# junliu111/CV-MonoSLAM

Measured on AMD Instinct MI355X. Metric: srukf_updates_per_sec, higher is better.
Workload: dtype f64; 1 GPU; BASELINE configs[2]: 200 inverse-depth landmarks (n=1204, Na=1209, L=2419), M=N matched, fp64, one batched refactor per frame, synthetic 640x480 figure-8 sequence; landmarks=200, state_dim=1204, sequences_per_gpu=1, update_mode=batched

## Files before the change

cv-monoslam_amd/csrc/srukf_api.hip:

```cpp

#include "srukf_ctx.h"
using namespace srukf_impl;


namespace srukf_impl {

void srukf_pool_init()
{
    static std::mutex mu;
    static unsigned long long done_mask = 0;
    int dev = 0; hipMemPool_t pool = nullptr;
    if (hipGetDevice(&dev) != hipSuccess || dev < 0 || dev >= 64) return;
    const unsigned long long bit = 1ull << dev;
    std::lock_guard<std::mutex> lk(mu);
    if (done_mask & bit) return;
    if (hipDeviceGetDefaultMemPool(&pool, dev) == hipSuccess && pool) {
        unsigned long long keep = ~0ull;
        hipMemPoolSetAttribute(pool, hipMemPoolAttrReleaseThreshold, &keep);
    }
    done_mask |= bit;
}

hipError_t srukf_dmalloc_raw(void** p, size_t bytes)
{
// ... 97 lines not shown
}

void host_weights(int Na, const srukf_params& p, KWeights& w)
{
    const double alpha = p.ut_alpha, beta = p.ut_beta;
    const double Lammda = alpha * alpha * Na - Na;
    switch (p.weight_type) {
    case 0:
        w.wm0 = 1.0 - Na / 3.0; w.wc0 = 1.0 - Na / 3.0; w.wi = (1.0 - w.wc0) / (2 * Na); w.wi_sr = sqrt(w.wi);
        w.gamma = sqrt(Na / (1.0 - w.wm0));
        break;
    case 1:
        w.gamma = sqrt(Na + Lammda); w.wm0 = Lammda / (Na + Lammda); w.wc0 = w.wm0 + (1 - alpha * alpha + beta);
        w.wi = 1.0 / (2 * (Na + Lammda)); w.wi_sr = sqrt(fabs(w.wi));
        break;
    default:
        w.gamma = sqrt(3.0 * Na / 2.0); w.wm0 = 1.0 / 3.0; w.wc0 = 1.0 / 3.0; w.wi = 1.0 / (3.0 * Na); w.wi_sr = sqrt(w.wi);
        break;
    }
}

void prof_collect(srukf_ctx* c)
{
    for (auto& e : c->pev) {
        float ms = 0.f;
        hipEventSynchronize(e.b);
        hipEventElapsedTime(&ms, e.a, e.b);
        c->prof_ms[e.kc] += ms; c->prof_n[e.kc] += 1;
        hipEventDestroy(e.a); hipEventDestroy(e.b);
    }
    c->pev.clear();
}

}


namespace srukf_impl {

std::vector<int> build_tile_table(int n_own, int n_other, bool upper, bool own_is_row, int k_index )
{
    std::vector<std::vector<int>> lst(8);
    for (int x = 0; x < 8; x++)
        for (int o = 0; o < n_other; o++)
            for (int w = x; w < n_own; w += 8) {
                const int r = own_is_row ? w : o, c = own_is_row ? o : w;
                if (upper && c < r) continue;
                lst[x].push_back(r); lst[x].push_back(c);
            }
    {
        for (auto& l : lst) {
            std::vector<std::pair<int, int>> t;
            for (size_t q = 0; q < l.size() / 2; q++) t.push_back({ l[2 * q], l[2 * q + 1] });
            std::stable_sort(t.begin(), t.end(), [k_index](const std::pair<int, int>& a, const std::pair<int, int>& b) {
                return k_index ? a.second > b.second : a.first > b.first; });
            for (size_t q = 0; q < t.size(); q++) { l[2 * q] = t[q].first; l[2 * q + 1] = t[q].second; }
        }
    }
    size_t mx = 0;
    for (auto& l : lst) mx = l.size() / 2 > mx ? l.size() / 2 : mx;
    std::vector<int> tab(mx * 8 * 2, -1);
    for (int x = 0; x < 8; x++)
        for (size_t q = 0; q < lst[x].size() / 2; q++) { tab[(q * 8 + x) * 2] = lst[x][2 * q]; tab[(q * 8 + x) * 2 + 1] = lst[x][2 * q + 1]; }
    return tab;
}

}

static int alloc_zero(srukf_ctx* c, void** p, size_t bytes)
{
    HIPCHK(c, srukf_dmalloc_on(p, bytes, c->stream));
    HIPCHK(c, hipMemsetAsync(*p, 0, bytes, c->stream));
    return SRUKF_OK;
}

#define ALLOC(ptr, count) do { int rc_ = alloc_zero(c, (void**)&(ptr), sizeof(*(ptr)) * (size_t)(count)); if (rc_) { g_create_error = c->err; srukf_destroy(c); return rc_; } } while (0)

static int block_cov(srukf_ctx* c, int off, int bs, double* out)
{
    srukf_launch_block_cov(c->stream, c->d, c->S, off, bs, c->small, nullptr);
    HIPCHK(c, hipMemcpyAsync(c->hstage, c->small, sizeof(double) * bs * bs, hipMemcpyDeviceToHost, c->stream));
    HIPCHK(c, hipStreamSynchronize(c->stream));
    memcpy(out, c->hstage, sizeof(double) * bs * bs);
    return SRUKF_OK;
}

extern "C" {

int srukf_abi_version(void) { return SRUKF_ABI_VERSION; }

int srukf_default_params(srukf_params* p)
{
    if (!p) return SRUKF_ERR_BAD_ARG;
    memset(p, 0, sizeof *p);
    p->cam_dx = 0.0028; p->cam_dy = 0.0028; p->cam_cx = 310.1129; p->cam_cy = 236.7526;
    p->cam_k1 = 0.0001; p->cam_k2 = 0.0; p->cam_f = 2.1735; p->image_w = 640; p->image_h = 480;
    p->a1 = p->a2 = p->a3 = p->a4 = 8.0; p->sigma_measure = 3.0; p->rho0 = 1.0 / 3.0; p->sigma_rho = p->rho0 / 2.0;
    p->sigma_x = 0.02; p->sigma_y = 0.02; p->sigma_z = 0.005; p->sigma_theta = 0.02;
    p->epsilon = 1e-13; p->ut_alpha = 1e-3; p->ut_beta = 2.0;
    p->weight_type = 0; p->noise_type = 0; p->newton_iters = 100;
    return SRUKF_OK;
}

const char* srukf_last_error(const srukf_ctx* ctx) { return ctx ? ctx->err.c_str() : g_create_error.c_str(); }

int srukf_create(srukf_ctx** out, int N, const srukf_params* p, int device, void* stream)
{
    if (!out || !p || N < 0) { g_create_error = "bad argument"; return SRUKF_ERR_BAD_ARG; }
    if (N > 32 * SRUKF_STAT_GROUPS) { g_create_error = "more than 2048 landmarks: the per-group statistics counters (FrameScalars::stat_cnt) serve 64 groups of 32"; return SRUKF_ERR_UNSUPPORTED; }
    if (p->noise_type != 0) { g_create_error = "noise_type != 0 draws random numbers (SLAM.cpp:1505-1516) and is not built"; return SRUKF_ERR_UNSUPPORTED; }
    int ndev = 0;
    if (hipGetDeviceCount(&ndev) != hipSuccess || ndev <= 0 || device < 0 || device >= ndev) {
        g_create_error = "no HIP device (this library has no CPU fallback)";
        return SRUKF_ERR_NO_DEVICE;
    }
    if (hipSetDevice(device) != hipSuccess) { g_create_error = "hipSetDevice failed"; return SRUKF_ERR_NO_DEVICE; }
    hipDeviceProp_t prop;
    if (hipGetDeviceProperties(&prop, device) != hipSuccess) { g_create_error = "hipGetDeviceProperties failed"; return SRUKF_ERR_NO_DEVICE; }
    if (strncmp(prop.gcnArchName, "gfx950", 6) != 0) {
        g_create_error = std::string("device is ") + prop.gcnArchName + ", kernels are built for gfx950 only";
        return SRUKF_ERR_NO_DEVICE;
    }
    srukf_ctx* c = new srukf_ctx();
    c->device = device; c->p = *p;
    if (!g_dbg_graphs) c->use_graph = false;
    memset(c->prof_ms, 0, sizeof c->prof_ms); memset(c->prof_n, 0, sizeof c->prof_n);
    memset(c->prof_flops, 0, sizeof c->prof_flops); memset(c->prof_bytes, 0, sizeof c->prof_bytes);
    if (stream) { c->stream = (hipStream_t)stream; c->own_stream = false; }
    else {
        if (hipStreamCreateWithFlags(&c->stream, hipStreamNonBlocking) != hipSuccess) { g_create_error = "hipStreamCreate failed"; delete c; return SRUKF_ERR_HIP; }
        c->own_stream = true;
    }
    KDims& d = c->d;
    d.N = N; d.n = 6 * N + 4; d.Na = d.n + 5; d.L = 2 * d.Na + 1;
    d.np = round_up(d.n, SRUKF_PAD); d.mp = round_up(2 * N > 0 ? 2 * N : 1, SRUKF_PAD);
    host_weights(d.Na, c->p, c->w);
    const size_t np = d.np, mp = d.mp;
    ALLOC(c->X, np); ALLOC(c->S, np * np); ALLOC(c->G, np * np); ALLOC(c->Gbak, np * np); ALLOC(c->Wf, np * np);
    ALLOC(c->sigR, (size_t)d.L * 8 + 8); ALLOC(c->mpart, srukf_meas_part_doubles(d.mp)); ALLOC(c->dxp, srukf_gain_part_doubles(d.np)); ALLOC(c->Cmat, (np + 64) * 4); ALLOC(c->Z, (size_t)d.L * mp); ALLOC(c->DZ, np * mp);
    ALLOC(c->Ut, mp * np); ALLOC(c->PxyR, 5 * mp);
    { const size_t Nn = (size_t)(N > 0 ? N : 1); ALLOC(c->h, mp + 4 * Nn + (Nn + 1) / 2); c->Si = c->h + mp; c->vis = (int*)(c->h + mp + 4 * Nn);
      ALLOC(c->zcur, mp + (Nn + 1) / 2); c->mcur = (int*)(c->zcur + mp); }
    ALLOC(c->D, np); ALLOC(c->odocur, 8); ALLOC(c->small, 64);
    ALLOC(c->theta, np); ALLOC(c->fs, 1);
    { char* pb0 = nullptr; char* pb1 = nullptr; ALLOC(pb0, srukf_gmw_panel_bytes()); ALLOC(pb1, srukf_gmw_panel_bytes()); c->pan[0] = pb0; c->pan[1] = pb1; }
    { const int rcg = gmw_plan_create(c->gplan, d.np, c->stream); if (rcg) { g_create_error = "persistent GMW resources: allocation failed"; srukf_destroy(c); return rcg; } }
    split_ensure(c, c->gplan);
    {
        std::vector<int> ts = build_tile_table(d.np / 32, d.np / 32, true, true, 0);
        std::vector<int> tp = build_tile_table(d.np / 32, d.mp / 32, false, false, 1);
        c->n_syrk_tiles = (int)ts.size() / 2; c->n_pxy_tiles = (int)tp.size() / 2;
        ALLOC(c->syrk_tiles, ts.size()); ALLOC(c->pxy_tiles, tp.size());
        std::vector<int> th;
        const int hd = srukf_gmw_head_rows(), hx = hd + 64 * srukf_gmw_head_extra_diag();
        for (int pass = 0; pass < 2; pass++)
            for (size_t q = 0; q + 1 < ts.size(); q += 2) {
                if (!(ts[q] >= 0 && (ts[q] * 32 < hd || (ts[q] * 32 < hx && ts[q + 1] * 32 < hx)))) continue;
                const bool crit = ts[q] * 32 < 128 && ts[q + 1] * 32 < 128;
                if (crit == (pass == 0)) { th.push_back(ts[q]); th.push_back(ts[q + 1]); }
            }
        c->n_syrk_head_crit = 0;
        for (size_t q = 0; q + 1 < th.size(); q += 2) if (th[q] * 32 < 128 && th[q + 1] * 32 < 128) c->n_syrk_head_crit++;
        c->n_syrk_head_tiles = (int)th.size() / 2;
        ALLOC(c->syrk_head_tiles, th.size() ? th.size() : 2);
        {
            std::vector<int> qx[8], tb;
            for (size_t q = 0; q + 1 < th.size(); q += 2) { const int x = (th[q + 1] / 2) % 8; qx[x].push_back(th[q]); qx[x].push_back(th[q + 1]); }
            size_t longest = 0;
            for (int x = 0; x < 8; x++) longest = std::max(longest, qx[x].size() / 2);
            for (size_t rnd = 0; rnd < longest; rnd++)
                for (int x = 0; x < 8; x++) { tb.push_back(2 * rnd + 1 < qx[x].size() ? qx[x][2 * rnd] : -1); tb.push_back(2 * rnd + 1 < qx[x].size() ? qx[x][2 * rnd + 1] : -1); }
            c->n_syrk_head_tiles_b = (int)tb.size() / 2;
            ALLOC(c->syrk_head_tiles_b, tb.size() ? tb.size() : 2);
            if (!tb.empty() && hipMemcpyAsync(c->syrk_head_tiles_b, tb.data(), sizeof(int) * tb.size(), hipMemcpyHostToDevice, c->stream) != hipSuccess) {
                g_create_error = "tile table upload failed"; srukf_destroy(c); return SRUKF_ERR_HIP;
            }
            if (hipStreamSynchronize(c->stream) != hipSuccess) { g_create_error = "tile table upload failed"; srukf_destroy(c); return SRUKF_ERR_HIP; }
        }
        if (!th.empty() && hipMemcpyAsync(c->syrk_head_tiles, th.data(), sizeof(int) * th.size(), hipMemcpyHostToDevice, c->stream) != hipSuccess) {
            g_create_error = "tile table upload failed"; srukf_destroy(c); return SRUKF_ERR_HIP;
        }
        if (hipMemcpyAsync(c->syrk_tiles, ts.data(), sizeof(int) * ts.size(), hipMemcpyHostToDevice, c->stream) != hipSuccess ||
            hipMemcpyAsync(c->pxy_tiles, tp.data(), sizeof(int) * tp.size(), hipMemcpyHostToDevice, c->stream) != hipSuccess ||
            hipStreamSynchronize(c->stream) != hipSuccess) {
            g_create_error = "tile table upload failed"; srukf_destroy(c); return SRUKF_ERR_HIP;
        }
    }
    c->hstage_bytes = sizeof(double) * (np * np + 4096);
    if (g_spare_stage && g_spare_stage_bytes >= c->hstage_bytes) {
        c->hstage = g_spare_stage; c->hstage_bytes = g_spare_stage_bytes; g_spare_stage = nullptr; g_spare_stage_bytes = 0;
    }
    if ((!c->hstage && hipHostMalloc((void**)&c->hstage, c->hstage_bytes) != hipSuccess) || hipHostMalloc((void**)&c->hfs, sizeof(FrameScalars) + sizeof(double) * (40 + c->d.mp + 5 * (size_t)c->d.N + 8)) != hipSuccess) {
        g_create_error = "hipHostMalloc failed"; srukf_destroy(c); return SRUKF_ERR_NOMEM;
    }
    memset(c->hfs, 0, sizeof(FrameScalars) + sizeof(double) * 40);
    c->hmeas = (double*)((char*)c->hfs + sizeof(FrameScalars) + sizeof(double) * 40);
    int rc = srukf_reset(c);
    if (rc) { g_create_error = c->err; srukf_destroy(c); return rc; }
    srukf_warm_exact_path(c->stream, c->fs);
    *out = c;
    return SRUKF_OK;
}

int srukf_destroy(srukf_ctx* c)
{
    if (!c) return SRUKF_OK;
    hipSetDevice(c->device);
    for (srukf_ctx* r : c->retired) srukf_destroy(r);
    c->retired.clear();
    if (c->spare_stage) { hipHostFree(c->spare_stage); c->spare_stage = nullptr; c->spare_stage_bytes = 0; }
    batch_plan_forget(c);
    if (c->stream) hipStreamSynchronize(c->stream);
    if (c->ck_stream) hipStreamSynchronize(c->ck_stream);
    if (c->side) hipStreamSynchronize(c->side);
    prof_collect(c);
    if (c->graph_exec) hipGraphExecDestroy(c->graph_exec);
    if (c->graph) hipGraphDestroy(c->graph);
    if (c->graph8_exec) hipGraphExecDestroy(c->graph8_exec);
    if (c->graph8) hipGraphDestroy(c->graph8);
    if (c->graphN_exec) hipGraphExecDestroy(c->graphN_exec);
    if (c->graphN) hipGraphDestroy(c->graphN);
    void* bufs[] = { c->X, c->S, c->G, c->Gbak, c->Wf, c->sigR, c->Cmat, c->Z, c->DZ, c->Ut, c->h , c->PxyR, c->D,
                     c->zcur , c->odocur, c->small, c->theta, c->fs, c->odo_seq, c->z_seq, c->m_seq, c->pan[0], c->pan[1], c->mpart, c->dxp, c->syrk_tiles, c->pxy_tiles, c->syrk_head_tiles,
                     c->perm, c->iperm, c->Sdis, c->ckS, c->ckX, c->ckS2, c->ckX2, c->odo_step, c->export_cnt, c->red_perm, c->red_iperm, c->gdiag, c->red_syrk_tiles, c->syrk_head_tiles_b, c->red_head0_tiles, c->split_fold_list, c->shadowA, c->Utp, c->P1, c->pxy2_tiles, c->nskip, c->slabW, c->slabL, c->gsW, c->gsL, c->S32, c->X32, c->U32, c->mx_part, c->mx_tasks, c->mx_tiles, c->fold_sync, c->dxk, c->A32, c->mxr_part, c->mxr_tasks, c->mxr_tiles, c->mxr_f64_tiles, c->mxr_xt, c->app_patch, c->app_tmpl, c->d_image, c->appR, c->appT, c->appPx, c->corr, c->has_app };
    for (void* b : bufs) if (b) srukf_dfree_on(b, c->stream);
    det_scratch_free(c->det, c->stream);
    gmw_plan_destroy(c->gplan, c->stream);
    gmw_plan_destroy(c->gplan_red, c->stream);
    if (c->side) { hipStreamSynchronize(c->side); hipStreamDestroy(c->side); hipEventDestroy(c->ev_fork); hipEventDestroy(c->ev_join); }
    if (c->ck_stream) { hipStreamSynchronize(c->ck_stream); hipStreamDestroy(c->ck_stream); hipEventDestroy(c->ck_e1); hipEventDestroy(c->ck_e2); if (c->ck_e3) hipEventDestroy(c->ck_e3); }
    if (c->own_stream && c->stream) hipStreamSynchronize(c->stream);
    if (c->hstage) {
        if (!g_spare_stage || g_spare_stage_bytes < c->hstage_bytes) { if (g_spare_stage) hipHostFree(g_spare_stage); g_spare_stage = c->hstage; g_spare_stage_bytes = c->hstage_bytes; }
        else hipHostFree(c->hstage);
    }
    if (c->hfs) hipHostFree(c->hfs);
    if (c->hview) hipHostFree(c->hview);
    if (c->own_stream && c->stream) hipStreamDestroy(c->stream);
    delete c;
    return SRUKF_OK;
}

}

namespace srukf_impl {

void ctx_retire(srukf_ctx* handle, srukf_ctx* old)
{
    drop_graphs(old);
    old->own_stream = false;
    if (old->hstage) {
        if (!handle->spare_stage || handle->spare_stage_bytes < old->hstage_bytes) {
            if (handle->spare_stage) hipHostFree(handle->spare_stage);
            handle->spare_stage = old->hstage; handle->spare_stage_bytes = old->hstage_bytes;
        } else hipHostFree(old->hstage);
        old->hstage = nullptr; old->hstage_bytes = 0;
    }
    handle->retired.push_back(old);
    const double ctx_bytes = 14.0 * 8.0 * (double)old->d.np * old->d.np;
    const size_t keep = (size_t)std::min((double)g_dbg_ctx_keep.load(), std::max(4.0, 16e9 / ctx_bytes));
    while (handle->retired.size() > keep) { srukf_destroy(handle->retired.front()); handle->retired.erase(handle->retired.begin()); }
}

static int ctx_revive(srukf_ctx* r)
{
    if (r->ck_stream) HIPCHK(r, hipStreamSynchronize(r->ck_stream));
    if (r->side) HIPCHK(r, hipStreamSynchronize(r->side));
    r->ck_pending = false; r->ck3_inflight = false; r->ck_valid = false;
    if (r->odo_seq) { srukf_dfree_on(r->odo_seq, r->stream); srukf_dfree_on(r->z_seq, r->stream); srukf_dfree_on(r->m_seq, r->stream); r->odo_seq = nullptr; r->z_seq = nullptr; r->m_seq = nullptr; }
    r->seqF = 0;
    r->storage = SRUKF_STORAGE_F64;
    r->K_new = 0; r->dx_pending = false; r->dx_lm = false; r->xr1_pending = false;
    if (r->fold_sync) HIPCHK(r, hipMemsetAsync(r->fold_sync, 0, sizeof(unsigned int) * (size_t)srukf_fold_words(r->d.mp / 64, r->d.np / 64), r->stream));
    r->null_canonical = false; r->tail_ok = false;
    r->clamp_frame_host = r->clamp_row_host = -1;
    r->next_odo_valid = false; r->fs_seq_step = false; r->last_update_sequential = false;
    r->step_export_attached = false; r->step_export = StepExport{}; r->mirror_next = false; r->meas_seq = 0;
    r->view_auto = false; r->view_unused = 0; r->view_hits = 0;
    r->step_fast_frames = r->step_slow_frames = 0; r->exact_frames = 0;
    r->profiling = false; r->pev.clear();
    r->err.clear();
    HIPCHK(r, hipMemsetAsync(r->fs, 0, sizeof(FrameScalars), r->stream));
    return srukf_reset(r);
}

int ctx_obtain(srukf_ctx* handle, srukf_ctx** out, int N)
{
    for (size_t q = 0; q < handle->retired.size(); q++) {
        srukf_ctx* r = handle->retired[q];
        if (r->d.N != N || r->device != handle->device || r->stream != handle->stream || memcmp(&r->p, &handle->p, sizeof(srukf_params)) != 0) continue;
        handle->retired.erase(handle->retired.begin() + (long)q);
        if (!r->hstage) {
            const size_t need = sizeof(double) * ((size_t)r->d.np * r->d.np + 4096);
            if (handle->spare_stage && handle->spare_stage_bytes >= need) { r->hstage = handle->spare_stage; r->hstage_bytes = handle->spare_stage_bytes; handle->spare_stage = nullptr; handle->spare_stage_bytes = 0; }
            else if (hipHostMalloc((void**)&r->hstage, need) == hipSuccess) r->hstage_bytes = need;
            else { r->hstage = nullptr; srukf_destroy(r); break; }
        }
        if (ctx_revive(r) == SRUKF_OK) { *out = r; return SRUKF_OK; }
        srukf_destroy(r);
        break;
    }
    if (handle->spare_stage && !g_spare_stage) { g_spare_stage = handle->spare_stage; g_spare_stage_bytes = handle->spare_stage_bytes; handle->spare_stage = nullptr; handle->spare_stage_bytes = 0; }
    return srukf_create(out, N, &handle->p, handle->device, handle->stream);
}

}

extern "C" {

int srukf_reset(srukf_ctx* c)
{
    if (!c) return SRUKF_ERR_BAD_ARG;
    HIPCHK(c, hipSetDevice(c->device));
    const KDims& d = c->d;
    const size_t np = d.np;
    step_state_replaced(c);
    HIPCHK(c, hipMemsetAsync(c->X, 0, sizeof(double) * np, c->stream));
    HIPCHK(c, hipMemsetAsync(c->S, 0, sizeof(double) * np * np, c->stream));
    double* hs = c->hstage;
    hs[0] = c->p.sigma_x; hs[1] = c->p.sigma_y; hs[2] = c->p.sigma_z; hs[3] = c->p.sigma_theta;
// ... 300 lines not shown
```

cv-monoslam_amd/csrc/srukf_ctx.h:

```cpp
#pragma once
#include <hip/hip_runtime.h>
#include <math.h>
#include <stdio.h>
#include <stdlib.h>
#include <string.h>
#include <string>
#include <cstddef>
#include <vector>
#include <algorithm>
#include <utility>
#include <atomic>
#include <mutex>
#include <map>
#include "srukf_device.h"
#include "srukf_rank.h"

extern "C" {
void srukf_launch_motion(hipStream_t, KDims, KWeights, srukf_params, double*, double*, double*, double*, FrameScalars*, const double*, const double*, RankArgs);
void srukf_launch_project(hipStream_t, KDims, KWeights, srukf_params, const double*, const double*, const double*, double*, double*, const FrameScalars*);
void srukf_launch_meas_stats(hipStream_t, KDims, KWeights, const double*, const double*, const double*, double*, double*, double*, int*, double*);
int srukf_meas_part_doubles(int);
void srukf_launch_gain(hipStream_t, KDims, KWeights, double*, const double*, const double*, const int*, const double*, const double*,
                       const double*, const int*, const int*, FrameScalars*, double*, double*, const double*, RankArgs, const double*, double*,
                       const double*, int, const double*, double, const double*, int, const double*, double*);
void srukf_launch_project_motion(hipStream_t, KDims, KWeights, srukf_params, double*, double*, double*, double*, double*, double*, FrameScalars*, RankArgs);
int srukf_gain_part_doubles(int);
void srukf_launch_traj(hipStream_t, KDims, const double*, const double*, FrameScalars*, double*, int);
void srukf_launch_block_cov(hipStream_t, KDims, const double*, int, int, double*, const double*);
void srukf_launch_project_points(hipStream_t, srukf_params, int, const double*, const double*, const double*, const double*, double*);
void srukf_launch_pxy(hipStream_t, KDims, const double*, const double*, double*, const void*, int, KWeights, MeasArgs);
void srukf_launch_pxy2(hipStream_t, KDims, const double*, const double*, double*, double*, const void*, int, int, KWeights, MeasArgs, GainFold);
int srukf_pxy2_build_tiles(int mp, int np, int kr, int* out);
int srukf_pxy2_split_groups(void);
void srukf_launch_syrk(hipStream_t, KDims, const double*, const double*, int, int, double*, FrameScalars*, const void*, int, const double*, double*, RankArgs, const double*);
void srukf_launch_gmw_step64(hipStream_t, int, int, int, double, double*, const void*, void*, double*, double*, const FrameScalars*);
int srukf_gmw_panel_bytes(void);
int srukf_gmw_sync_bytes(int T);
int srukf_gmw_build_tiles(int T, int Tp, short* out);
int srukf_gmw_persist_workers(int T, int Tp, int max_workers);
void srukf_launch_gmw_persist(hipStream_t, int, int, double, double*, void*, double*, double*, void*, const void*, int, int, void*, const double*, const double*, int, int, int, int, int);
void srukf_launch_gmw_persist_head(hipStream_t, int, int, double, double*, void*, double*, double*, void*, const void*, int, int, void*, const double*, const double*, int, int, int, int, int, const HeadArgs*);
void srukf_launch_gmw_split(hipStream_t, hipStream_t, int, int, double, double*, void*, double*, double*, void*, const void*, int, void*, int, int, double*, double*, int);
void srukf_launch_gmw_split_fold(hipStream_t, hipStream_t, int, int, double, double*, void*, double*, double*, void*, const void*, int, void*, int, int, double*, double*, const double*, const double*, int);
int srukf_gmw_build_fold_list(int T, int Tp, short* out);
int srukf_gmw_fold_head_tile(int tr, int tc, int head_rows);
int srukf_gmw_fold_head_rows(int Tp);
void srukf_gmw_fold_head_override(int v);
void srukf_launch_gmw_split_alone(hipStream_t, int, int, int, double, double*, void*, double*, double*, void*, const void*, int, void*, int, int, double*, double*);
void srukf_launch_row_energy(hipStream_t, int, int, const double*, double*);
void srukf_launch_rank_diag(hipStream_t, int, int, const double*, const int*, double*);
void srukf_launch_rank_expand(hipStream_t, int, int, int, double, const double*, const double*, const int*, const int*, const double*, void*, const double*, int, double*, double*, double*, double, int, KDims, KWeights, srukf_params, double*, double*, int, const StepExport*, double, unsigned int*, int);
void srukf_launch_project_table(hipStream_t, KDims, KWeights, srukf_params, double*, double*, double*, double*, double*, double*, FrameScalars*, RankArgs, NullSkip);
void srukf_launch_sigr_rows(hipStream_t, KDims, KWeights, const double*, const double*, double*, const FrameScalars*, const int*, int);
void srukf_launch_rank_shadow(hipStream_t, int, int, int, const double*, const int*, double*);
void srukf_launch_rank_canon(hipStream_t, int, int, int, double, const int*, double*);
void srukf_launch_rank_round(hipStream_t, int, int, double*);
void srukf_launch_syrk_own(hipStream_t, int, int, const double*, const double*, int, int, int, double*, void*, const void*, int, int);
int srukf_gmw_register_form(int, int, int, int);
int srukf_pxy2_b_per(int, int);
void srukf_launch_pxy2_b(hipStream_t, KDims, const void*, int, const void*, int, int, KWeights, int);
void srukf_launch_gain_b(hipStream_t, KDims, KWeights, const void*, int, int, double);
void srukf_launch_syrk_b(hipStream_t, KDims, const void*, int, const void*, int, int, int, int);
void srukf_launch_syrk_own_b(hipStream_t, int, int, const void*, int, int, int, int, const void*, int, int);
void srukf_launch_gmw_step64_b(hipStream_t, int, int, int, double, const void*, int, int, int);
void srukf_launch_gmw_pivslab_b(hipStream_t, int, int, int, double, const void*, int, int, int);
void srukf_launch_gmw_trail_b(hipStream_t, int, int, const void*, int, int, int, int);
void srukf_launch_rank_expand_b(hipStream_t, int, int, int, double, const void*, int, double, KDims, KWeights, srukf_params);
int srukf_gmw_head_rows(void);
int srukf_gmw_head_extra_diag(void);
void srukf_launch_gmw_check(hipStream_t, int, int, const double*, const double*, FrameScalars*, const double*, int, double*);
void srukf_launch_gmw_col(hipStream_t, int, int, int, double, const double*, double*, double*, unsigned long long*, FrameScalars*, double*);
void srukf_set_exact_right_looking(int on);
void srukf_warm_exact_path(hipStream_t st, FrameScalars* fs);
int srukf_get_exact_right_looking(void);
void srukf_launch_gmw_stats(hipStream_t, int, int, const double*, FrameScalars*);
void srukf_launch_landmarks_cartesian(hipStream_t, KDims, const double*, const double*, double*, double*);
void srukf_launch_aug_map(hipStream_t, srukf_params, int, int, int, int, double, const double*, const double*, const double*, double*);
void srukf_launch_aug_x(hipStream_t, int, int, int, double, double, const double*, const double*, const int*, double*, double*, int, int);
void srukf_launch_aug_build(hipStream_t, int, int, int, int, double, double, const double*, const double*, const double*, double*, int, int, int);
void srukf_launch_gram(hipStream_t, int, int, const double*, double*);
void srukf_launch_warp_patch(hipStream_t, KDims, srukf_params, const double*, const double*, const double*, const double*, const double*, const double*,
                             const unsigned char*, const int*, unsigned char*);
void srukf_launch_associate(hipStream_t, KDims, srukf_params, const unsigned char*, const double*, const double*, const int*, const int*,
                            const unsigned char*, double*, int*, double*);
int srukf_mixed_build_tasks(int np, int ue, short* out_tasks, int* out_tiles, int* ntiles);
int srukf_mixed_build_tasks_red(int np, int ue, int krows, int rows_lim, short* out_tasks, int* out_tiles, int* ntiles);
int srukf_mixed_krows(int r);
void srukf_launch_split_bf3(hipStream_t, int, int, int, int, const double*, void*, size_t);
void srukf_launch_syrk_bf3(hipStream_t, int, int, int, int, int, const void*, size_t, const void*, int, const void*, int, double*, double*, void*);
size_t srukf_mixed_part_bytes(int ntasks);
void srukf_launch_cvt_f32(hipStream_t, size_t, const double*, float*);
void srukf_launch_cvt_robot_cols(hipStream_t, int, int, const double*, float*);
void srukf_launch_gain_dx(hipStream_t, int, int, const double*, double*, const double*);
void srukf_launch_syrk32(hipStream_t, int, int, int, const float*, const float*, const void*, int, const void*, int, double*, double*, void*, int);
int srukf_app_patch_stride(void);
int srukf_app_tmpl_stride(void);
}

#define SRUKF_GRAPH_FRAMES 8
#define SRUKF_MAX_TENANTS 4
#define SRUKF_NULL_ENERGY 1e-12
#ifndef SRUKF_BATCH_GROUPS_MAX
#define SRUKF_BATCH_GROUPS_MAX 4
#endif

enum KClass { KC_MOTION = 0, KC_PROJECT, KC_STATS, KC_PXY, KC_GAIN, KC_SYRK, KC_GMW_TRAIL, KC_GMW_PERSIST, KC_GMW_CHECK,
              KC_GMW_COL, KC_RANK_EXPAND, KC_PROJECT_MOTION, KC_PROJECT_TABLE, KC_PXY2, KC_MISC,
              KC_DET_RESPONSE, KC_DET_CAND, KC_DET_RANK, KC_DET_SELECT, KC_CAPTURE, KC_COUNT };
struct ProfEvent { hipEvent_t a, b; int kc; };

struct GmwPlan { void* pans = nullptr; void* sync = nullptr; void* tiles = nullptr; int ntiles = 0, nreal = 0, T = 0, Tp = 0, workers = -1, tenants = 1, cus = 0; };

struct DetScratch {
    double *resp = nullptr, *cand_r = nullptr; int *cand_pix = nullptr, *sorted = nullptr, *rank = nullptr, *gxy = nullptr, *blk = nullptr; void* hdr = nullptr;
    void *in = nullptr, *out = nullptr; size_t in_bytes = 0, out_bytes = 0;
};

struct srukf_ctx {
    int device = 0;
    hipStream_t stream = nullptr;
    bool own_stream = false;
    srukf_params p;
    KDims d;
    KWeights w;
    double *X = nullptr, *S = nullptr, *G = nullptr, *Gbak = nullptr, *Wf = nullptr;
    double *sigR = nullptr, *Cmat = nullptr, *Z = nullptr, *DZ = nullptr, *Ut = nullptr;
    double *h = nullptr, *Si = nullptr, *PxyR = nullptr, *D = nullptr;
    double *zcur = nullptr, *odocur = nullptr, *small = nullptr, *mpart = nullptr, *dxp = nullptr;
    int *vis = nullptr, *mcur = nullptr;
    unsigned long long* theta = nullptr;
    bool dx_pending = false;
    bool dx_lm = false;
    unsigned int* fold_sync = nullptr; double* dxk = nullptr; int fold_robot_tiles = 0;
    bool xr1_pending = false;
    int K_new = 0;
    unsigned char *app_patch = nullptr, *app_tmpl = nullptr, *d_image = nullptr;
    double *appR = nullptr, *appT = nullptr, *appPx = nullptr, *corr = nullptr;
    int* has_app = nullptr;
    bool frame_valid = false;
    DetScratch det;
    int storage = SRUKF_STORAGE_F64;
    float *S32 = nullptr, *X32 = nullptr;
    float *U32 = nullptr; double* mx_part = nullptr; void *mx_tasks = nullptr, *mx_tiles = nullptr; int mx_ntasks = 0, mx_ntiles = 0;
    float* A32 = nullptr; double* mxr_part = nullptr; void *mxr_tasks = nullptr, *mxr_tiles = nullptr; int mxr_ntasks = 0, mxr_ntiles = 0, mxr_krows = 0, mxr_for_r = 0;
    int* mxr_f64_tiles = nullptr; int mxr_n_f64_tiles = 0;
    unsigned short* mxr_xt = nullptr; size_t mxr_xt_stride = 0; int mxr_ktot = 0;
    int *perm = nullptr, *iperm = nullptr;
    double* Sdis = nullptr;
    void* pan[2] = { nullptr, nullptr };
    GmwPlan gplan;
    int red_r = 0, red_Tp = 0;
    int rank_aware = 1;
    int *red_perm = nullptr, *red_iperm = nullptr;
    double* gdiag = nullptr;
    double *shadowA = nullptr, *Utp = nullptr;
    double *slabW = nullptr, *slabL = nullptr;
    double *gsW = nullptr, *gsL = nullptr; int gs_panels = 0;
    hipStream_t side = nullptr; hipEvent_t ev_fork = nullptr, ev_join = nullptr;
    bool split_off = false;
    double* P1 = nullptr; int* pxy2_tiles = nullptr; int n_pxy2_tiles = 0, pxy2_split_b0 = 0;
    int* nskip = nullptr; int ns_full = 0, ns_null = 0, ns_rows = 0;
    int* red_head0_tiles = nullptr; int n_red_head0_tiles = 0;
    void* split_fold_list = nullptr; int n_split_fold = 0;
    double red_head0_flop = 0.0;
    int* red_syrk_tiles = nullptr; int n_red_syrk_tiles = 0;
    double red_fac_flop = 0, red_own_flop = 0;
    GmwPlan gplan_red;
    int shared_tenants = 2;
    int gmw_shared = 0;
    int debug_allow_mixed = 0;
    struct DbgSwitches {
        int fused_motion = 2;
        int f32_fuse = 1;
        int table_perm = 1;
        int tail_fuse = 1;
        int head_fold = 1;
        int nullskip = 1;
        int pxy2 = 1;
        int step_fuse_export = 1;
        int view_auto = 1;
        int step_early = 2;
        int step_spin = 1;
        int step_fast = 1;
        int split_record = 0;
        int null_canon = 1;
        int split_fold = 1;
        int gain_fold = 0;
        int mixed_rank = 1;
        int mixed_null_ppm = 1;
        int mixed_bf16 = 0;
        int mixed_f64_robot = 1;
    } dbg;
    bool null_canonical = false;
    bool tail_ok = false;
    int debug_starve = 0;
    int clamp_frame_host = -1, clamp_row_host = -1;
    double *ckS = nullptr, *ckX = nullptr;
    int *syrk_tiles = nullptr, *pxy_tiles = nullptr;
    int *syrk_head_tiles = nullptr;
    int n_syrk_tiles = 0, n_pxy_tiles = 0, n_syrk_head_tiles = 0, n_syrk_head_crit = 0;
    int* syrk_head_tiles_b = nullptr; int n_syrk_head_tiles_b = 0;
    FrameScalars* fs = nullptr;
    int seqF = 0;
    double *odo_seq = nullptr, *z_seq = nullptr;
    int* m_seq = nullptr;
    double* hstage = nullptr; size_t hstage_bytes = 0;
    FrameScalars* hfs = nullptr;
    double* hmeas = nullptr;
    int phase = 0;
    double next_odo[6] = { 0, 0, 0, 0, 0, 0 }; bool next_odo_valid = false;
    double* odo_step = nullptr;
    double step_odo[6] = { 0, 0, 0, 0, 0, 0 };
    int step_seqF = 1;
    bool step_fast = false;
    bool step_uncommitted = false;
    bool step_chain = false;
    bool proj_valid = false; double proj_odo[6] = { 0, 0, 0, 0, 0, 0 };
    bool fs_seq_step = false;
    bool last_update_sequential = false;
    double *ckS2 = nullptr, *ckX2 = nullptr; hipEvent_t ck_e3 = nullptr; bool ck_valid = false;
    bool ck3_inflight = false;
    unsigned spin_ok = 0;
    bool pre_issued = false; double pre_odo[6] = { 0, 0, 0, 0, 0, 0 };
    bool next_pose_pending = false;
    bool setstep_done = false; double setstep_odo[6] = { 0, 0, 0, 0, 0, 0 };
    hipStream_t ck_stream = nullptr; hipEvent_t ck_e1 = nullptr, ck_e2 = nullptr; bool ck_pending = false;
    unsigned long long meas_seq = 0;
    bool step_export_attached = false;
    int* export_cnt = nullptr;
    StepExport step_export = {};
    bool mirror_next = false;
    unsigned long long step_seq = 0;
    double* hview = nullptr; size_t hview_doubles = 0;
    bool view_auto = false; int view_unused = 0;
    int view_hits = 0;
    bool view_cached = false;
    bool robot_cached = false;
    bool f32_stale = false;
    int step_fast_frames = 0, step_slow_frames = 0;
    double* spare_stage = nullptr; size_t spare_stage_bytes = 0;
    int split_fold_seqs = 0;
    int fold_seqs = 0;
    int exact_frames = 0;
    bool async_pending = false;
    std::vector<srukf_ctx*> retired;
    std::string err;
    hipGraph_t graph = nullptr, graph8 = nullptr;
    hipGraphExec_t graph_exec = nullptr, graph8_exec = nullptr;
    hipGraph_t graphN = nullptr; hipGraphExec_t graphN_exec = nullptr; int graphN_frames = 0;
    bool use_graph = true;
    bool profiling = false;
    std::vector<ProfEvent> pev;
    double prof_ms[KC_COUNT]; long long prof_n[KC_COUNT]; double prof_flops[KC_COUNT]; double prof_bytes[KC_COUNT];
};

#define HIPCHK(ctx, call) do { hipError_t e_ = (call); if (e_ != hipSuccess) { \
    char b_[256]; snprintf(b_, sizeof b_, "%s failed: %s (%s:%d)", #call, hipGetErrorString(e_), __FILE__, __LINE__); \
    (ctx)->err = b_; return SRUKF_ERR_HIP; } } while (0)

namespace srukf_impl {

inline bool storage_f32_like(const srukf_ctx* c) { return c->storage == SRUKF_STORAGE_F32 || (c->storage == SRUKF_STORAGE_F32_MIXED && c->dbg.mixed_rank && c->A32); }

extern const char* const kclass_name[KC_COUNT];
extern thread_local std::string g_create_error;
extern std::atomic<int> g_dbg_gmw_persist, g_dbg_gmw_fused, g_dbg_rank_fused, g_dbg_rank_fold, g_dbg_rank_aware, g_dbg_graphs, g_dbg_mem_split, g_dbg_shared_tenants;
extern std::atomic<int> g_dbg_batch_wide, g_dbg_batch_groups, g_dbg_batch_split, g_dbg_head_fold_free;
extern std::atomic<int> g_dbg_timing, g_dbg_fold_head, g_dbg_fold_force, g_dbg_ctx_keep, g_dbg_batch_xcd, g_dbg_batch_k128;

inline int round_up(int v, int m) { return (v + m - 1) / m * m; }

void srukf_pool_init();
hipError_t srukf_dmalloc_raw(void** p, size_t bytes);
template <class T> inline hipError_t srukf_dmalloc(T** p, size_t bytes) { return srukf_dmalloc_raw((void**)p, bytes); }
hipError_t srukf_dfree(void* p);
template <class T> inline hipError_t srukf_dmalloc_on(T** p, size_t bytes, hipStream_t st) { srukf_pool_init(); return hipMallocAsync((void**)p, bytes ? bytes : 8, st); }
hipError_t srukf_dfree_on(void* p, hipStream_t st);

void launch_refactor_reset(hipStream_t st, int np, unsigned long long* theta_bits, FrameScalars* fs, int reset_stats);
void launch_set_seq(hipStream_t st, FrameScalars* fs, const double* odo_seq, int seqF, double a1, double a2, double a3, double a4);
void launch_set_frame(hipStream_t st, FrameScalars* fs, int frame, int clear_clamp);
void launch_set_traj(hipStream_t st, FrameScalars* fs, double* traj_base);
void launch_set_run(hipStream_t st, FrameScalars* fs, int frame, int clear_clamp, double* traj_base);
void launch_set_step(hipStream_t st, FrameScalars* fs, double* odo, int seqF, double a1, double a2, double a3, double a4, int fresh, const double poses[9]);
void launch_export(hipStream_t st, const void* a, size_t bytes_a, const void* b, size_t bytes_b, void* host_pinned, unsigned long long* flag = nullptr, unsigned long long seq = 0);
void launch_set_frame_control(hipStream_t st, FrameScalars* fs);
void launch_commit_motion(hipStream_t st, int n, int ld, double* X, double* S, const double* Cm, const FrameScalars* fs, double* A, const int* iperm, int rk);
void launch_sym_permute(hipStream_t st, int n, int ld, const double* src, int lds, double* dst, const int* map);
void launch_gather(hipStream_t st, int n, int ld, const double* src, double* dst, const int* map);
void launch_zero_rows(hipStream_t st, int ld, int r0, double* A);
void launch_quantize(hipStream_t st, int n, int ld, double* S, double* X, float* S32, float* X32);

void gmw_plan_destroy(GmwPlan& g, hipStream_t st = nullptr);
int gmw_plan_create(GmwPlan& g, int np, hipStream_t st, int Tp = 0, int tenants = 1);
void host_weights(int Na, const srukf_params& p, KWeights& w);
std::vector<int> build_tile_table(int n_own, int n_other, bool upper, bool own_is_row, int k_index );
void prof_collect(srukf_ctx* c);
void adopt_context(srukf_ctx* c, srukf_ctx* c2);
int ctx_obtain(srukf_ctx* handle, srukf_ctx** out, int N);
void ctx_retire(srukf_ctx* handle, srukf_ctx* old);

void det_scratch_free(DetScratch& s, hipStream_t st);
int ensure_image(srukf_ctx* c);
int take_frame(srukf_ctx* c, const unsigned char* gray);
void launch_capture_patch(hipStream_t st, const unsigned char* img, int W, int first, int K, const double* uv, const double* X, int n,
                          unsigned char* app_patch, unsigned char* app_tmpl, double* appR, double* appT, double* appPx, int* has_app);

#define SRUKF_LM_RECORD_DOUBLES 113
void launch_lm_record(hipStream_t st, const double* P66, const double* X, int k, double eps, const unsigned char* app_patch, const double* appR,
                      const double* appT, const double* appPx, const int* has_app, double* out);
void launch_lm_insert(hipStream_t st, const double* S, int ld, const double* X, int p6, int L, const double* blk, double* S2, double* X2, int n2, int ld2);

struct ProfScope {
    srukf_ctx* c; int kc; hipEvent_t a = nullptr, b = nullptr;
    ProfScope(srukf_ctx* c_, int kc_, double flops, double bytes) : c(c_), kc(kc_) {
        if (c->profiling) {
            hipEventCreate(&a); hipEventCreate(&b); hipEventRecord(a, c->stream);
            c->prof_flops[kc] += flops; c->prof_bytes[kc] += bytes;
        }
    }
    ~ProfScope() {
        if (c->profiling) { hipEventRecord(b, c->stream); c->pev.push_back({ a, b, kc }); }
    }
};

void step_commit_motion(srukf_ctx* c);
unsigned long long* step_flag(srukf_ctx* c);
int step_wait_export(srukf_ctx* c, unsigned long long seq);
void step_invalidate(srukf_ctx* c);
void step_state_replaced(srukf_ctx* c);
void step_ck_join(srukf_ctx* c);

void quantize_state(srukf_ctx* c);
RankArgs rank_args(const srukf_ctx* c, bool prep_next = false, bool dzperm = false, bool f32round = false);
NullSkip null_skip(const srukf_ctx* c);
const double* take_xr1(srukf_ctx* c);
void seq_predict_fused(srukf_ctx* c, int mode);
void seq_predict_motion(srukf_ctx* c, const double* odo_pair_dev);
void seq_predict_measurement(srukf_ctx* c, bool fused_stats);
void shadow_rebuild(srukf_ctx* c);
bool gmw_plan_persists(const srukf_ctx* c, const GmwPlan& gp);
bool gmw_use_persist(const srukf_ctx* c);
int gmw_persist_mode();
int plan_tenants(const srukf_ctx* c);
int gate_limit(const srukf_ctx* c);
void rank_expand(srukf_ctx* c, bool frame_tail, bool table = false, bool fuse = false);
bool replay_red_fused(const srukf_ctx* c);
bool replay_red_perm(const srukf_ctx* c);
int replay_motion_mode(const srukf_ctx* c);
bool replay_fuse_mode(const srukf_ctx* c);
bool head_fold_ok(const srukf_ctx* c);
int gmw_fused_mode();
int rank_fused_mode();
// ... 29 lines not shown
```

cv-monoslam_amd/csrc/srukf_debug.hip:

```cpp

#include "srukf_ctx.h"
using namespace srukf_impl;


namespace srukf_impl {
std::atomic<int> g_dbg_gmw_persist{1}, g_dbg_gmw_fused{1}, g_dbg_rank_fused{1}, g_dbg_rank_fold{1}, g_dbg_rank_aware{1}, g_dbg_graphs{1};
std::atomic<int> g_dbg_mem_split{1};
std::atomic<int> g_dbg_shared_tenants{2};
std::atomic<int> g_dbg_batch_wide{1}, g_dbg_batch_groups{0}, g_dbg_batch_split{1};
std::atomic<int> g_dbg_timing{0}, g_dbg_fold_head{0}, g_dbg_fold_force{0}, g_dbg_ctx_keep{24}, g_dbg_batch_xcd{1}, g_dbg_batch_k128{1};
std::atomic<int> g_dbg_head_fold_free{0};
}

static bool debug_buffer(srukf_ctx* c, const char* key, double** ptr, long long* cap)
{
    const KDims& d = c->d;
    const GmwPlan& gp = c->red_r > 0 ? c->gplan_red : c->gplan;
    double* src = nullptr; long long n = 0;
    if (!strcmp(key, "Z")) { src = c->Z; n = (long long)d.L * d.mp; }
    else if (!strcmp(key, "DZ")) { src = c->DZ; n = (long long)d.np * d.mp; }
    else if (!strcmp(key, "sigR")) { src = c->sigR; n = (long long)(d.L + 1) * 8; }
    else if (!strcmp(key, "Cmat")) { src = c->Cmat; n = (long long)d.n * 4; }
    else if (!strcmp(key, "Xr1")) { src = (double*)((char*)c->fs + offsetof(FrameScalars, Xr1)); n = 4; }
    else if (!strcmp(key, "Utp")) { src = c->Utp; n = c->Utp ? (long long)d.mp * d.np : 0; }
    else if (!strcmp(key, "P1")) { src = c->P1; n = c->P1 ? (long long)d.mp * d.np : 0; }
    else if (!strcmp(key, "h")) { src = c->h; n = 2LL * d.N; }
    else if (!strcmp(key, "Si")) { src = c->Si; n = 4LL * d.N; }
    else if (!strcmp(key, "det_resp")) { src = c->det.resp; n = c->det.resp ? (long long)c->p.image_w * (long long)c->p.image_h : 0; }
    else if (!strcmp(key, "Wf")) { src = c->Wf; n = (long long)d.np * d.np; }
    else if (!strcmp(key, "Gbak")) { src = c->Gbak; n = (long long)d.np * d.np; }
    else if (!strcmp(key, "G")) { src = c->G; n = (long long)d.np * d.np; }
    else if (!strcmp(key, "D")) { src = c->D; n = d.np; }
    else if (!strcmp(key, "fold_dbg")) { src = c->fold_sync ? (double*)(c->fold_sync + ((srukf_fold_words(d.mp / 64, d.np / 64) + 1) & ~1)) : nullptr; n = c->fold_sync ? FOLD_DBG_STAMPS : 0; }
    else if (!strcmp(key, "gsW")) { src = c->gsW; n = c->gsW ? (long long)c->gs_panels * 64 * d.np : 0; }
    else if (!strcmp(key, "gsL")) { src = c->gsL; n = c->gsL ? (long long)c->gs_panels * 64 * d.np : 0; }
    else if (!strcmp(key, "pans")) { src = (double*)gp.pans; n = gp.pans ? (long long)srukf_gmw_panel_bytes() * gp.T / 8 : 0; }
    else if (!strcmp(key, "sync")) { src = (double*)gp.sync; n = gp.sync ? (long long)srukf_gmw_sync_bytes(gp.T) / 8 : 0; }
    else return false;
    *ptr = src; *cap = n;
    return true;
}

extern "C" {

int srukf_debug_allow_mixed(srukf_ctx* c, int on)
{
    if (!c) return SRUKF_ERR_BAD_ARG;
    c->debug_allow_mixed = on ? 1 : 0;
    return SRUKF_OK;
}

int srukf_debug_poke_state(srukf_ctx* c, int row, int col, double value)
{
    if (!c || row < 0 || col < row || col >= c->d.n) return SRUKF_ERR_BAD_ARG;
    HIPCHK(c, hipSetDevice(c->device));
    step_commit_motion(c); step_invalidate(c);
    HIPCHK(c, hipStreamSynchronize(c->stream));
    HIPCHK(c, hipMemcpy(c->S + (size_t)row * c->d.np + col, &value, sizeof(double), hipMemcpyHostToDevice));
    return SRUKF_OK;
}

int srukf_debug_set(srukf_ctx* c, const char* key, int value)
{
    if (!key) return SRUKF_ERR_BAD_ARG;
    struct { const char* k; std::atomic<int>* v; } globals[] = { { "gmw_persist", &g_dbg_gmw_persist }, { "gmw_fused", &g_dbg_gmw_fused }, { "rank_fused", &g_dbg_rank_fused },
                                                    { "rank_fold", &g_dbg_rank_fold }, { "rank_aware", &g_dbg_rank_aware }, { "graphs", &g_dbg_graphs }, { "mem_split", &g_dbg_mem_split }
                                                  };
    if (!strcmp(key, "batch_split")) { g_dbg_batch_split = value ? 1 : 0; batch_drop_all_graphs(); return SRUKF_OK; }
    if (!strcmp(key, "head_fold_free")) { if (value < 1) return SRUKF_ERR_BAD_ARG; g_dbg_head_fold_free = value; if (c) { hipSetDevice(c->device); step_commit_motion(c); step_invalidate(c); hipStreamSynchronize(c->stream); drop_graphs(c); } return SRUKF_OK; }
    if (!strcmp(key, "batch_groups")) { if (value < 0 || value > SRUKF_BATCH_GROUPS_MAX) return SRUKF_ERR_BAD_ARG; g_dbg_batch_groups = value; return SRUKF_OK; }
    if (!strcmp(key, "batch_wide")) { g_dbg_batch_wide = value ? 1 : 0; return SRUKF_OK; }
    if (!strcmp(key, "timing")) { g_dbg_timing = value ? 1 : 0; return SRUKF_OK; }
    if (!strcmp(key, "fold_head")) { g_dbg_fold_head = value < 0 ? 0 : value; srukf_gmw_fold_head_override(g_dbg_fold_head); return SRUKF_OK; }
    if (!strcmp(key, "batch_k128")) { g_dbg_batch_k128 = value ? 1 : 0; batch_drop_all_graphs(); return SRUKF_OK; }
    if (!strcmp(key, "batch_xcd")) { g_dbg_batch_xcd = value ? 1 : 0; batch_drop_all_graphs(); return SRUKF_OK; }
    if (!strcmp(key, "ctx_keep")) { g_dbg_ctx_keep = value < 0 ? 0 : value; return SRUKF_OK; }
    if (!strcmp(key, "fold_force")) { g_dbg_fold_force = value ? 1 : 0; return SRUKF_OK; }
    if (!strcmp(key, "exact_rl")) { srukf_set_exact_right_looking(value); return SRUKF_OK; }
    if (!strcmp(key, "shared_tenants")) {
        if (value < 2 || value > 8) return SRUKF_ERR_BAD_ARG;
        g_dbg_shared_tenants = value;
        return SRUKF_OK;
    }
    for (auto& g : globals)
        if (!strcmp(key, g.k)) {
            g.v->store(!strcmp(key, "mem_split") ? value : (value ? 1 : 0));
            if (c) { hipSetDevice(c->device); step_commit_motion(c); step_invalidate(c); hipStreamSynchronize(c->stream); drop_graphs(c); if (!strcmp(key, "rank_aware")) return update_null_set(c); }
            return SRUKF_OK;
        }
    if (!c) return SRUKF_ERR_BAD_ARG;
    HIPCHK(c, hipSetDevice(c->device));
    step_commit_motion(c); step_invalidate(c);
    HIPCHK(c, hipStreamSynchronize(c->stream));
    if (!strcmp(key, "use_graph")) c->use_graph = value != 0;
    else if (!strcmp(key, "pxy2")) c->dbg.pxy2 = value ? 1 : 0;
    else if (!strcmp(key, "nullskip")) c->dbg.nullskip = value ? 1 : 0;
    else if (!strcmp(key, "head_fold")) c->dbg.head_fold = value ? 1 : 0;
    else if (!strcmp(key, "tail_fuse")) c->dbg.tail_fuse = value ? 1 : 0;
    else if (!strcmp(key, "table_perm")) c->dbg.table_perm = value ? 1 : 0;
    else if (!strcmp(key, "f32_fuse")) c->dbg.f32_fuse = value ? 1 : 0;
    else if (!strcmp(key, "split_record")) c->dbg.split_record = value ? 1 : 0;
    else if (!strcmp(key, "gain_fold")) c->dbg.gain_fold = value ? 1 : 0;
    else if (!strcmp(key, "null_canon")) c->dbg.null_canon = value ? 1 : 0;
    else if (!strcmp(key, "split_fold")) c->dbg.split_fold = value < 0 ? 0 : value > 2 ? 2 : value;
    else if (!strcmp(key, "mixed_rank")) c->dbg.mixed_rank = value ? 1 : 0;
    else if (!strcmp(key, "mixed_f64_robot")) c->dbg.mixed_f64_robot = value ? 1 : 0;
    else if (!strcmp(key, "mixed_bf16")) c->dbg.mixed_bf16 = value ? 1 : 0;
    else if (!strcmp(key, "mixed_null_ppm")) c->dbg.mixed_null_ppm = value < 0 ? 0 : value;
    else if (!strcmp(key, "step_fast")) c->dbg.step_fast = value ? 1 : 0;
    else if (!strcmp(key, "step_spin")) c->dbg.step_spin = value ? 1 : 0;
    else if (!strcmp(key, "step_early")) c->dbg.step_early = value < 0 ? 0 : value > 2 ? 2 : value;
    else if (!strcmp(key, "view_auto")) { c->dbg.view_auto = value ? 1 : 0; if (!value) { c->view_auto = false; c->view_cached = false; } }
    else if (!strcmp(key, "step_fuse_export")) c->dbg.step_fuse_export = value ? 1 : 0;
    else if (!strcmp(key, "fused_motion")) c->dbg.fused_motion = value < 0 ? 0 : value > 2 ? 2 : value;
    else { c->err = std::string("srukf_debug_set: unknown key ") + key; return SRUKF_ERR_BAD_ARG; }
    drop_graphs(c);
    return SRUKF_OK;
}

int srukf_debug_gmw_stamps(srukf_ctx* c, unsigned long long* buf)
{
    if (!c) return SRUKF_ERR_BAD_ARG;
    static unsigned long long* dbuf = nullptr;
    HIPCHK(c, hipSetDevice(c->device));
    HIPCHK(c, hipStreamSynchronize(c->stream));
    GmwPlan& g = c->red_r > 0 ? c->gplan_red : c->gplan;
    if (!g.sync) return SRUKF_ERR_SEQUENCE;
    if (!dbuf) { HIPCHK(c, hipMalloc((void**)&dbuf, 8 * 4096)); HIPCHK(c, hipMemset(dbuf, 0, 8 * 4096)); }
    if (buf) HIPCHK(c, hipMemcpy(buf, dbuf, 8 * 4096, hipMemcpyDeviceToHost));
    HIPCHK(c, hipMemcpy((char*)g.sync + offsetof(GmwSync, dbg), &dbuf, 8, hipMemcpyHostToDevice));
    return SRUKF_OK;
}

int srukf_debug_get(srukf_ctx* c, const char* key, long long* value)
{
    if (!c || !key || !value) return SRUKF_ERR_BAD_ARG;
    HIPCHK(c, hipSetDevice(c->device));
    HIPCHK(c, hipMemcpyAsync(c->hfs, c->fs, sizeof(FrameScalars), hipMemcpyDeviceToHost, c->stream));
    HIPCHK(c, hipStreamSynchronize(c->stream));
    if (!strcmp(key, "gmw_aborts")) *value = c->hfs->gmw_aborts;
    else if (!strcmp(key, "clamp_rows")) *value = c->hfs->clamp_rows;
    else if (!strcmp(key, "frame")) *value = c->hfs->frame;
    else if (!strcmp(key, "frozen")) *value = c->hfs->frozen;
    else if (!strcmp(key, "gate_timeouts")) *value = c->hfs->gate_timeouts;
    else if (!strcmp(key, "gmw_shared")) *value = c->gmw_shared;
    else if (!strcmp(key, "split_off")) *value = c->split_off ? 1 : 0;
    else if (!strncmp(key, "pad", 3) && key[3] >= '1' && key[3] <= '7' && !key[4]) {
        const GmwPlan& gp = c->red_r > 0 ? c->gplan_red : c->gplan;
        unsigned long long v = 0, zero = 0;
        const size_t off = offsetof(GmwSync, pad) + 8 * (size_t)(key[3] - '0');
        if (gp.sync) { HIPCHK(c, hipMemcpy(&v, (char*)gp.sync + off, sizeof v, hipMemcpyDeviceToHost)); HIPCHK(c, hipMemcpy((char*)gp.sync + off, &zero, sizeof zero, hipMemcpyHostToDevice)); }
        *value = (long long)v;
    }
    else if (!strcmp(key, "abort_code")) {
        const GmwPlan& gp = c->red_r > 0 ? c->gplan_red : c->gplan;
        unsigned long long code = 0, zero = 0;
        if (gp.sync) {
            HIPCHK(c, hipMemcpy(&code, (char*)gp.sync + offsetof(GmwSync, pad), sizeof code, hipMemcpyDeviceToHost));
            HIPCHK(c, hipMemcpy((char*)gp.sync + offsetof(GmwSync, pad), &zero, sizeof zero, hipMemcpyHostToDevice));
        }
        *value = (long long)code;
    }
    else if (!strcmp(key, "step_fast")) *value = c->step_fast_frames;
    else if (!strcmp(key, "step_slow")) *value = c->step_slow_frames;
    else if (!strcmp(key, "exact_frames")) *value = c->exact_frames;
    else if (!strcmp(key, "fold_seqs")) *value = c->fold_seqs;
    else if (!strcmp(key, "split_fold_seqs")) *value = c->split_fold_seqs;
    else if (!strncmp(key, "pxy2_stamp", 10) && key[10] >= '1' && key[10] <= '7') { const unsigned long long* t = (const unsigned long long*)(c->hmeas + c->d.mp + 5 * (size_t)c->d.N); *value = (long long)(t[key[10] - '0'] - t[0]); }
    else if (!strcmp(key, "meas_flag_ticks")) { const unsigned long long* t = (const unsigned long long*)(c->hmeas + c->d.mp + 5 * (size_t)c->d.N); *value = (long long)(t[1] - t[0]); }
    else if (!strcmp(key, "view_hits")) *value = c->view_hits;
    else if (!strcmp(key, "view_auto")) *value = c->view_auto ? 1 : 0;
    else if (!strcmp(key, "split_form")) *value = split_form(c, c->red_r > 0 ? c->gplan_red : c->gplan) ? 1 : 0;
    else if (!strncmp(key, "plan_", 5)) {
        const GmwPlan& gp = c->red_r > 0 ? c->gplan_red : c->gplan;
        const bool persist = gmw_use_persist(c) && gmw_plan_persists(c, gp);
        const char* k = key + 5;
        if (!strcmp(k, "T")) *value = gp.T;
        else if (!strcmp(k, "Tp")) *value = gp.Tp;
        else if (!strcmp(k, "tiles")) *value = gp.nreal;
        else if (!strcmp(k, "workers")) *value = gp.workers;
        else if (!strcmp(k, "persist")) *value = persist ? 1 : 0;
        else if (!strcmp(k, "register_form")) *value = (persist && !split_form(c, gp) && srukf_gmw_register_form(gp.T, gp.Tp, gp.ntiles, gp.workers)) ? 1 : 0;
        else if (!strcmp(k, "tiles_per_worker")) *value = gp.workers > 0 ? (gp.nreal + gp.workers - 1) / gp.workers : -1;
        else if (!strcmp(k, "fold")) *value = replay_red_fused(c) ? 1 : 0;
        else if (!strcmp(k, "head_fold")) *value = (replay_red_fused(c) && head_fold_ok(c)) ? 1 : 0;
        else if (!strcmp(k, "red_perm")) *value = (!replay_red_fused(c) && replay_red_perm(c)) ? 1 : 0;
        else if (!strcmp(k, "motion")) *value = replay_motion_mode(c);
        else if (!strcmp(k, "fuse")) *value = replay_fuse_mode(c) ? 1 : 0;
        else if (!strcmp(k, "kept")) *value = c->red_r;
        else if (!strcmp(k, "sync_doubles")) *value = gp.sync ? srukf_gmw_sync_bytes(gp.T) / 8 : 0;
        else if (!strcmp(k, "pans_doubles")) *value = gp.pans ? (long long)srukf_gmw_panel_bytes() * gp.T / 8 : 0;
        else if (!strcmp(k, "slab_panels")) *value = c->gs_panels;
        else return SRUKF_ERR_BAD_ARG;
    }
    else return SRUKF_ERR_BAD_ARG;
    return SRUKF_OK;
}

int srukf_debug_copy(srukf_ctx* c, const char* key, double* out, long long count)
{
    if (!c || !key || !out || count < 0) return SRUKF_ERR_BAD_ARG;
    HIPCHK(c, hipSetDevice(c->device));
    HIPCHK(c, hipStreamSynchronize(c->stream));
    double* src = nullptr; long long cap = 0;
    if (!debug_buffer(c, key, &src, &cap)) return SRUKF_ERR_BAD_ARG;
    if (!src || count > cap) return SRUKF_ERR_DIM_MISMATCH;
    HIPCHK(c, hipMemcpy(out, src, sizeof(double) * (size_t)count, hipMemcpyDeviceToHost));
    return SRUKF_OK;
}

int srukf_debug_upload(srukf_ctx* c, const char* key, const double* in, long long count)
{
    if (!c || !key || !in || count < 0) return SRUKF_ERR_BAD_ARG;
    HIPCHK(c, hipSetDevice(c->device));
    HIPCHK(c, hipStreamSynchronize(c->stream));
    double* dst = nullptr; long long cap = 0;
    if (!debug_buffer(c, key, &dst, &cap)) return SRUKF_ERR_BAD_ARG;
    if (!dst || count > cap) return SRUKF_ERR_DIM_MISMATCH;
    HIPCHK(c, hipMemcpy(dst, in, sizeof(double) * (size_t)count, hipMemcpyHostToDevice));
    return SRUKF_OK;
}

int srukf_debug_starve_workers(srukf_ctx* c, int on)
{
    if (!c) return SRUKF_ERR_BAD_ARG;
    c->debug_starve = on == 2 ? 2 : on ? 1 : 0;
    step_invalidate(c);
    drop_graphs(c);
    return SRUKF_OK;
}

int srukf_gmw_host(int device, int n, const double* G, double* S_out, double* D_out, double epsilon, int force_slow, int* clamp_hit)
{
    if (n < 1 || !G || !S_out) return SRUKF_ERR_BAD_ARG;
    int ndev = 0;
    if (hipGetDeviceCount(&ndev) != hipSuccess || device < 0 || device >= ndev) return SRUKF_ERR_NO_DEVICE;
    if (hipSetDevice(device) != hipSuccess) return SRUKF_ERR_NO_DEVICE;
    const int np = round_up(n, SRUKF_PAD);
    const size_t bytes = sizeof(double) * (size_t)np * np;
    std::vector<double> hG((size_t)np * np, 0.0), hS((size_t)np * np, 0.0), hD(np, 0.0);
    for (int r = 0; r < n; r++) for (int c = r; c < n; c++) hG[(size_t)r * np + c] = G[(size_t)r * n + c];
    struct Res {
        double *dG = nullptr, *dS = nullptr, *dD = nullptr, *dWf = nullptr; unsigned long long* dTh = nullptr; FrameScalars* dFs = nullptr;
        void* pan[2] = { nullptr, nullptr }; GmwPlan gp;
        ~Res() { for (void* b : { (void*)dG, (void*)dS, (void*)dD, (void*)dWf, (void*)dTh, (void*)dFs, pan[0], pan[1] }) if (b) srukf_dfree(b); gmw_plan_destroy(gp); }
    } r;
#define GH(call) do { if ((call) != hipSuccess) return SRUKF_ERR_HIP; } while (0)
    GH(srukf_dmalloc((void**)&r.dG, bytes)); GH(srukf_dmalloc((void**)&r.dS, bytes)); GH(srukf_dmalloc((void**)&r.dWf, bytes));
    GH(srukf_dmalloc((void**)&r.dD, sizeof(double) * np)); GH(srukf_dmalloc((void**)&r.dTh, sizeof(unsigned long long) * np)); GH(srukf_dmalloc((void**)&r.dFs, sizeof(FrameScalars)));
    GH(hipMemcpy(r.dG, hG.data(), bytes, hipMemcpyHostToDevice));
    GH(hipMemset(r.dS, 0, bytes)); GH(hipMemset(r.dWf, 0, bytes)); GH(hipMemset(r.dTh, 0, sizeof(unsigned long long) * np));
    GH(hipMemset(r.dFs, 0, sizeof(FrameScalars))); GH(hipMemset(r.dD, 0, sizeof(double) * np));
    hipStream_t st = nullptr;
    srukf_launch_gmw_stats(st, n, np, r.dG, r.dFs);
    FrameScalars fs;
    if (!force_slow) {
        if (gmw_persist_mode()) { const int rc = gmw_plan_create(r.gp, np, st); if (rc) return rc; }
        if (gmw_persist_mode() && r.gp.workers >= 0) {
            srukf_launch_gmw_persist(st, n, np, epsilon, r.dG, r.gp.pans, r.dD, r.dS, r.gp.sync, r.gp.tiles, r.gp.ntiles, r.gp.workers, r.dFs, nullptr, nullptr, 0, 0, 0, 0, 0);
        } else {
            GH(srukf_dmalloc(&r.pan[0], srukf_gmw_panel_bytes())); GH(srukf_dmalloc(&r.pan[1], srukf_gmw_panel_bytes()));
            GH(hipMemset(r.pan[0], 0, srukf_gmw_panel_bytes())); GH(hipMemset(r.pan[1], 0, srukf_gmw_panel_bytes()));
            int pb = 0;
            for (int j0 = -64; j0 + 64 < np; j0 += 64, pb ^= 1)
                srukf_launch_gmw_step64(st, n, np, j0, epsilon, r.dG, r.pan[pb ^ 1], r.pan[pb], r.dD, r.dS, nullptr);
        }
        GH(hipDeviceSynchronize());
        srukf_launch_gmw_check(st, n, np, r.dD, r.dS, r.dFs, nullptr, 0, nullptr);
        GH(hipMemcpy(&fs, r.dFs, sizeof fs, hipMemcpyDeviceToHost));
        if (clamp_hit) *clamp_hit = fs.clamp_rows;
        if (fs.clamp_rows > 0) force_slow = 2;
    }
    if (force_slow) {
        GH(hipMemcpy(r.dG, hG.data(), bytes, hipMemcpyHostToDevice));
        GH(hipMemset(r.dTh, 0, sizeof(unsigned long long) * np));
        GH(hipMemset(r.dS, 0, bytes));
        for (int j = 0; j < n; j++) srukf_launch_gmw_col(st, n, np, j, epsilon, r.dG, r.dWf, r.dD, r.dTh, r.dFs, r.dS);
        GH(hipMemcpy(&fs, r.dFs, sizeof fs, hipMemcpyDeviceToHost));
        if (clamp_hit && force_slow == 1) *clamp_hit = fs.clamp_rows;
    }
    GH(hipDeviceSynchronize());
    GH(hipMemcpy(hS.data(), r.dS, bytes, hipMemcpyDeviceToHost));
    GH(hipMemcpy(hD.data(), r.dD, sizeof(double) * np, hipMemcpyDeviceToHost));
#undef GH
    for (int rr = 0; rr < n; rr++) memcpy(S_out + (size_t)rr * n, hS.data() + (size_t)rr * np, sizeof(double) * n);
    if (D_out) memcpy(D_out, hD.data(), sizeof(double) * n);
    return SRUKF_OK;
}

int srukf_project_host(int device, const srukf_params* p, int count, const double* feat6, const double* pos3, const double* psi,
                       const double* err2, double* uv_out)
{
    if (!p || count < 1 || !feat6 || !pos3 || !psi || !err2 || !uv_out) return SRUKF_ERR_BAD_ARG;
    int ndev = 0;
    if (hipGetDeviceCount(&ndev) != hipSuccess || device < 0 || device >= ndev) return SRUKF_ERR_NO_DEVICE;
    if (hipSetDevice(device) != hipSuccess) return SRUKF_ERR_NO_DEVICE;
    double *df, *dp, *ds, *de, *dout;
    srukf_dmalloc((void**)&df, sizeof(double) * 6 * count); srukf_dmalloc((void**)&dp, sizeof(double) * 3 * count);
    srukf_dmalloc((void**)&ds, sizeof(double) * count); srukf_dmalloc((void**)&de, sizeof(double) * 2 * count); srukf_dmalloc((void**)&dout, sizeof(double) * 2 * count);
    hipMemcpy(df, feat6, sizeof(double) * 6 * count, hipMemcpyHostToDevice); hipMemcpy(dp, pos3, sizeof(double) * 3 * count, hipMemcpyHostToDevice);
    hipMemcpy(ds, psi, sizeof(double) * count, hipMemcpyHostToDevice); hipMemcpy(de, err2, sizeof(double) * 2 * count, hipMemcpyHostToDevice);
    srukf_launch_project_points(nullptr, *p, count, df, dp, ds, de, dout);
    hipError_t e = hipDeviceSynchronize();
    hipMemcpy(uv_out, dout, sizeof(double) * 2 * count, hipMemcpyDeviceToHost);
    srukf_dfree(df); srukf_dfree(dp); srukf_dfree(ds); srukf_dfree(de); srukf_dfree(dout);
    return e == hipSuccess ? SRUKF_OK : SRUKF_ERR_HIP;
}

}
```

cv-monoslam_amd/csrc/srukf_device.h:

```cpp
#pragma once
#include <hip/hip_runtime.h>
#include "../../include/srukf.h"

typedef double d4 __attribute__((ext_vector_type(4)));

#define SRUKF_NB 32
#define SRUKF_PAD 64

struct KDims {
    int N, n, Na, L;
    int np, mp;
};

struct KWeights { double wm0, wc0, wi, wi_sr, gamma; };

#define SRUKF_STAT_GROUPS 64
struct FrameScalars {
    double Ut[3];
    double Mt[3];
    double Xr0[4];
    unsigned long long gmax_bits;
    unsigned long long ximax_bits;
    int clamp_rows;
    int clamp_first;
// ... 148 lines not shown
    oy = vis ? vy : 0.0;
}

__device__ __forceinline__ void srukf_sigma_feat(const double (&base)[6], const double (&dev)[6], double e0, double e1, double gq,
                                                 double (&feat)[6], double& q0, double& q1)
{
#pragma clang fp contract(off)
#pragma unroll
    for (int e = 0; e < 6; e++) feat[e] = fma(dev[e], gq, base[e] * 1) + 0;
    q0 = fma(e0, gq, 0.0 * 1) + 0; q1 = fma(e1, gq, 0.0 * 1) + 0;
}
__device__ __forceinline__ void srukf_project_sigma(const srukf_params& p, double f1, double f2, const double (&base)[6], const double (&dev)[6],
                                                    double e0, double e1, double gq, const double* r, double& ox, double& oy)
{
    double feat[6], q0, q1;
    srukf_sigma_feat(base, dev, e0, e1, gq, feat, q0, q1);
    srukf_project(p, f1, f2, feat, r[0], r[1], r[2], r[4], r[5], q0, q1, ox, oy);
}

#define GAIN_SLICES 32
__device__ __forceinline__ void srukf_gain_dx_job(int n, int np, const double* __restrict__ dxp, double* __restrict__ X, int job, const double* xr1 = nullptr, int f32 = 0, int lmN = 0)
{
    const int r = job * 256 + threadIdx.x;
    if (r >= n) return;
    double acc = 0.0;
    if (lmN > 0) {
        const int per = (lmN + GAIN_SLICES - 1) / GAIN_SLICES;
        for (int u = 0; u < GAIN_SLICES; u++) {
            const int kb = u * per, cnt = min(lmN, kb + per) - kb;
            double s[4] = { 0.0, 0.0, 0.0, 0.0 };
            for (int q = 0; q < cnt; q++) s[q & 3] += dxp[(size_t)(kb + q) * np + r];
            acc += (s[0] + s[1]) + (s[2] + s[3]);
        }
    } else
#pragma unroll
    for (int u = 0; u < GAIN_SLICES; u++) acc += dxp[(size_t)u * np + r];
    const double x = (xr1 && r >= n - 4) ? xr1[r - (n - 4)] : X[r];
    double v = x + acc;
    if (f32) v = (double)(float)v;
    X[r] = v;
}

struct GainLm { double i00, i01, i10, i11, y0, y1; int on; };
__device__ __forceinline__ GainLm srukf_gain_lm(double s00, double s01, double s10, double s11, double z0, double z1, double h0, double h1, int on)
{
#pragma clang fp contract(off)
    GainLm g;
    double det = fma(s00, s11, -(s01 * s10));
    g.i00 = 0.0; g.i01 = 0.0; g.i10 = 0.0; g.i11 = 0.0;
    if (det != 0.0) { det = 1.0 / det; g.i00 = s11 * det; g.i01 = -s01 * det; g.i10 = -s10 * det; g.i11 = s00 * det; }
    const double v0 = z0 - h0, v1 = z1 - h1;
    g.y0 = fma(g.i10, v1, g.i00 * v0); g.y1 = fma(g.i11, v1, g.i01 * v0);
    g.on = on;
    return g;
}
__device__ __forceinline__ double srukf_gain_pxy(double q0, double q1, bool split, double dz, bool nullrow, double sqeps, double sc)
{
#pragma clang fp contract(off)
    double q = q0;
    if (split) q = q + q1;
    if (nullrow) q = fma(sqeps, dz, q);
    return sc * q;
}
__device__ __forceinline__ double srukf_gain_recentre(double p, double dxs, double s4, double hz, double rse)
{
#pragma clang fp contract(off)
    return fma(-hz, rse, fma(-dxs, s4, p));
}
__device__ __forceinline__ void srukf_gain_apply(const GainLm& g, double p0, double p1, double& u0, double& u1, double& c)
{
#pragma clang fp contract(off)
    u0 = fma(p1, g.i10, p0 * g.i00);
    u1 = fma(p1, g.i11, p0 * g.i01);
    c = fma(u1, g.y1, u0 * g.y0);
}

struct GainFold {
    unsigned int* sync;
    double* Utp; double* dxk;
    const double* z_seq; const int* m_seq;
    const double* DZp; const int* perm; const int* iperm; int r; int split_b0; double sqeps; double sc;
    double* S; double* A;
    int nmt, nbt, bt_r0, bt_r1, robot_tiles;
};
#define FOLD_FLAG_STRIDE 1024
#define FOLD_PAIR(mt, bt, nbt) (4 * ((mt) * (nbt) + (bt)))
__host__ __device__ inline int srukf_fold_flag_base(int nmt, int nbt) { return (4 * nmt * nbt + FOLD_FLAG_STRIDE - 1) / FOLD_FLAG_STRIDE * FOLD_FLAG_STRIDE; }
#define FOLD_MOTION(nmt, nbt) (srukf_fold_flag_base(nmt, nbt))
#define FOLD_ROBOT(nmt, nbt) (srukf_fold_flag_base(nmt, nbt) + FOLD_FLAG_STRIDE)
#define FOLD_STAT(g, nmt, nbt) (srukf_fold_flag_base(nmt, nbt) + FOLD_FLAG_STRIDE * (2 + (g)))
__host__ __device__ inline int srukf_fold_words(int nmt, int nbt) { return srukf_fold_flag_base(nmt, nbt) + FOLD_FLAG_STRIDE * (2 + SRUKF_STAT_GROUPS); }
#define FOLD_DBG_STAMPS 8192
#ifdef SRUKF_FOLD_DBG
#define FOLD_TS(gf, slot) do { if ((gf).sync && (threadIdx.x & 63) == 0) { unsigned long long t_; asm volatile("s_memrealtime %0\n\ts_waitcnt lgkmcnt(0)" : "=s"(t_) :: "memory"); \
    ((unsigned long long*)((gf).sync + ((srukf_fold_words((gf).nmt, (gf).nbt) + 1) & ~1)))[slot] = t_; } } while (0)
#else
#define FOLD_TS(gf, slot) do { } while (0)
#endif

struct NullSkip { const int* dirs; const int* nulls; const int* rows; int nfull, nnull, nrows; const int* iperm; int r; };

struct MeasArgs {
    const double* X; const double* xrob; const double* sigR; const double* Z; double* part;
    double* h; double* Si; int* vis; double* PxyR;
    FrameScalars* fs; int gx;
    NullSkip ns;
    int preamble;
    int fmode;
    double* Cm;
    char* hmirror; unsigned long long* hflag; unsigned long long hseq;
    unsigned long long* hstamp;
};

struct StepExport { unsigned long long* dst; int nfs; double* view; unsigned long long* flag; unsigned long long seq; int* cnt; int set; double* odo; double poses[6]; double a[4]; };
__device__ __forceinline__ void srukf_step_scalars(FrameScalars* fs, double* odo, int seqF, const double (&a)[4], bool clear_frozen = true)
{
    fs->odo_seq = odo; fs->seqF = seqF;
    fs->a[0] = a[0]; fs->a[1] = a[1]; fs->a[2] = a[2]; fs->a[3] = a[3];
    fs->frame = 0;
    fs->traj_base = nullptr;
    fs->stat_count = 0;
    for (int q = 0; q < SRUKF_STAT_GROUPS; q++) fs->stat_cnt[q] = 0;
    fs->clamp_rows = 0; fs->clamp_first = 0x7fffffff; fs->clamp_frame = 0x7fffffff; fs->gmw_aborts = 0;
    if (clear_frozen) fs->frozen = 0;
}

__device__ __forceinline__ double ld_dev(const double* p) { return __hip_atomic_load(p, __ATOMIC_RELAXED, __HIP_MEMORY_SCOPE_AGENT); }
__device__ __forceinline__ void st_dev(double* p, double v) { __hip_atomic_store(p, v, __ATOMIC_RELAXED, __HIP_MEMORY_SCOPE_AGENT); }
template <bool DEV> __device__ __forceinline__ double ld_g(const double* p) { if constexpr (DEV) return ld_dev(p); else return *p; }
template <bool DEV> __device__ __forceinline__ void st_d4(double* p, d4 v)
{
    if constexpr (DEV) { st_dev(p, v[0]); st_dev(p + 1, v[1]); st_dev(p + 2, v[2]); st_dev(p + 3, v[3]); }
    else *(d4*)p = v;
}

#define GMW_EPOCH_SHIFT 12
#define GMW_FLAG_COPIES 16
#define GMW_FLAG_STRIDE 512
struct GmwSync {
    unsigned long long epoch;
    unsigned int exited;
    int abort;
    unsigned long long* dbg;
    unsigned int head_done;
    unsigned int head_crit;
    unsigned int resident;
    unsigned int pad32;
    unsigned long long pad[59];
    unsigned long long panel_ready[GMW_FLAG_COPIES * GMW_FLAG_STRIDE];
    unsigned long long half_ready[GMW_FLAG_COPIES * GMW_FLAG_STRIDE];
};
__device__ __forceinline__ unsigned int* gmw_head_crit(GmwSync* sy) { return (unsigned int*)&sy->panel_ready[GMW_FLAG_STRIDE / 2]; }
__device__ __forceinline__ unsigned int* gmw_head_done(GmwSync* sy) { return (unsigned int*)&sy->half_ready[GMW_FLAG_STRIDE / 2]; }
__device__ __forceinline__ unsigned long long* gmw_sync_ver(GmwSync* sy) { return (unsigned long long*)(sy + 1); }
#define GMW_VER_STRIDE 16
#define GMW_VIDX(I, J, T) (((size_t)(I) * (T) + (J)) * GMW_VER_STRIDE)
__device__ __forceinline__ unsigned long long* gmw_sync_slabver(GmwSync* sy, int T) { return (unsigned long long*)(sy + 1) + (size_t)T * T * GMW_VER_STRIDE; }
__device__ __forceinline__ unsigned long long* gmw_sync_formver(GmwSync* sy, int T) { return (unsigned long long*)(sy + 1) + (size_t)2 * T * T * GMW_VER_STRIDE; }

#ifdef SRUKF_GMW_DBG
#define GMW_DBG(sy, slot, val) do { if (__builtin_amdgcn_readfirstlane(threadIdx.x >> 6) == 0 && (sy)->dbg) __hip_atomic_store(&(sy)->dbg[blockIdx.x * 8 + (slot)], (unsigned long long)(val), __ATOMIC_RELAXED, __HIP_MEMORY_SCOPE_SYSTEM); } while (0)
#define GMW_DBG2(sy, slot, val) do { if ((sy)->dbg) __hip_atomic_store(&(sy)->dbg[blockIdx.x * 8 + (slot)], (unsigned long long)(val), __ATOMIC_RELAXED, __HIP_MEMORY_SCOPE_SYSTEM); } while (0)
#define GMW_TS(sy, p, slot) do { if ((sy)->dbg) { unsigned long long t_; asm volatile("s_memrealtime %0\n\ts_waitcnt lgkmcnt(0)" : "=s"(t_) :: "memory"); (sy)->dbg[2048 + (p) * 8 + (slot)] = t_; } } while (0)
#else
#define GMW_DBG(sy, slot, val)
#define GMW_DBG2(sy, slot, val)
#define GMW_TS(sy, p, slot)
#endif

#ifdef SRUKF_STAMPS
__device__ unsigned long long srukf_stamps[32];
#define STAMP(i) do { if (blockIdx.x == 0 && blockIdx.y == 0 && threadIdx.x == 0) { unsigned long long t_; asm volatile("s_memtime %0\n\ts_waitcnt lgkmcnt(0)" : "=s"(t_) :: "memory"); srukf_stamps[i] = t_; } } while (0)
#define STAMPW(i) do { if (blockIdx.x == 0 && blockIdx.y == 0 && (threadIdx.x & 63) == 0) { unsigned long long t_; asm volatile("s_memtime %0\n\ts_waitcnt lgkmcnt(0)" : "=s"(t_) :: "memory"); srukf_stamps[i] = t_; } } while (0)
#else
#define STAMP(i)
#define STAMPW(i)
#endif

struct Step64Args { double* G; double* Sout; double* D; void* pan[2]; double* Wb; double* Lb; };
struct SyrkOwnArgs { const double* S0; const double* Ut0; double* G; FrameScalars* fs; };

struct LaunchCtx;
```

cv-monoslam_amd/csrc/srukf_gmw_persist.hip:

```cpp
#include <hip/hip_runtime.h>
#include <algorithm>
#include <cmath>
#include <cstdio>
#include <cstdlib>
#include <utility>
#include <vector>
#include "srukf_device.h"
#include "srukf_tiles.h"
#include "srukf_gmw_cols.h"
#include "srukf_gmw_panel.h"
#include "srukf_rank.h"

#ifndef GMW_XWG_LIMIT
#define GMW_XWG_LIMIT (1 << 16)
#endif
__device__ __forceinline__ unsigned long long gmw_uniform64(unsigned long long v)
{
    return ((unsigned long long)(unsigned)__builtin_amdgcn_readfirstlane((int)(v >> 32)) << 32) | (unsigned)__builtin_amdgcn_readfirstlane((int)v);
}
__device__ __forceinline__ bool gmw_wait_ge(const unsigned long long* f, unsigned long long want, const int* abort_flag)
{
    for (int spins = 0; spins < GMW_XWG_LIMIT; spins++) {
        if (gmw_uniform64(__hip_atomic_load(f, __ATOMIC_RELAXED, __HIP_MEMORY_SCOPE_AGENT)) >= want) return true;
        if ((spins & 31) == 31 && __builtin_amdgcn_readfirstlane(__hip_atomic_load(abort_flag, __ATOMIC_RELAXED, __HIP_MEMORY_SCOPE_AGENT))) return false;
        __builtin_amdgcn_s_sleep(1);
    }
    return false;
}
__device__ __forceinline__ void gmw_abandon(GmwSync* sy, unsigned int site)
{
    __hip_atomic_store(&sy->abort, 1, __ATOMIC_RELAXED, __HIP_MEMORY_SCOPE_AGENT);
    if ((threadIdx.x & 63) == 0) atomicCAS(&sy->pad[0], 0ull, ((unsigned long long)site << 32) | (unsigned long long)(blockIdx.x + 1));
}
__device__ __forceinline__ void gmw_set_flag(unsigned long long* f, unsigned long long v)
{
    __hip_atomic_store(f, v, __ATOMIC_RELAXED, __HIP_MEMORY_SCOPE_AGENT);
}
__device__ __forceinline__ void gmw_set_panel_flag(unsigned long long* f, unsigned long long v, int lane)
{
    if (lane < GMW_FLAG_COPIES) __hip_atomic_store(&f[lane * GMW_FLAG_STRIDE], v, __ATOMIC_RELAXED, __HIP_MEMORY_SCOPE_AGENT);
}
__device__ __forceinline__ void gmw_publish(unsigned long long* f, unsigned long long v, bool wv0)
{
    asm volatile("s_waitcnt vmcnt(0)" ::: "memory");
    __syncthreads();
    if (wv0) gmw_set_flag(f, v);
}

struct GmwPivotKeep {
    double* T1;
    double* T2;
    double* Ep;
    double* rD;
    double* sq;
};

__device__ __forceinline__ void gmw_stage_tile(double (*dst)[G64_LS], const double* __restrict__ G, int ld, int row0, int col0, int lane)
{
    const double* src = G + (size_t)row0 * ld + col0 + lane;
    double v[64];
#pragma unroll
    for (int r = 0; r < 64; r++) v[r] = ld_dev(src + (size_t)r * ld);
#pragma unroll
    for (int r = 0; r < 64; r++) dst[r][lane] = v[r];
}

__device__ __forceinline__ void gmw_pivot_persist(int n, int ld, int T, int Tp, double eps, double* __restrict__ G, GmwPanel64* __restrict__ pans,
                                                  double* __restrict__ Dall, double* __restrict__ Sout, GmwSync* sy, unsigned long long ebase,
                                                  double (*Lr)[G64_LS], double (*Wc)[G64_LS], double* facreg, double* xreg, double* keepreg,
                                                  int* okp, int* halfcnt, int* stageok, int tid, int klim)
{
    const int lane = tid & 63, wv = tid >> 6, lr = lane & 15, lk = lane >> 4;
    const int qa = wv >> 1, qb = wv & 1;
    const GmwColsLds ws = gmw_cols_carve(facreg), ws2 = gmw_cols_carve(facreg + GMW_FAC_DOUBLES);
    double (*X01)[32] = (double (*)[32])xreg;
    double (*X11)[32] = (double (*)[32])(xreg + 1024);
    GmwPivotKeep kp;
    kp.T1 = xreg + 2048; kp.T2 = xreg; kp.Ep = keepreg; kp.rD = keepreg + 1024; kp.sq = keepreg + 1088;
    unsigned long long* ver = gmw_sync_ver(sy);
    const int ro = (wv == 1) ? 0 : 32;
    const int wvu = __builtin_amdgcn_readfirstlane(wv);
    const bool wv0 = wvu == 0, wv1 = wvu == 1, wv3 = wvu == 3;
    if (wv0) *okp = 1;
    if (wv3) gmw_stage_tile(Wc, G, ld, 0, 0, lane);
    __syncthreads();
    for (int p = 0; p < Tp; p++) {
        const int j0 = 64 * (p - 1), base = 64 * p;
        const bool first = (p == 0);
        const bool half_only = (p == Tp - 1) && (Tp < T) && (klim <= base + 32);
        GmwPanel64* nxt = pans + p;
        if (wv0) GMW_TS(sy, p, 0);
        if (wv0) { ws.Dv[lane & 31] = 0.0; ws2.Dv[lane & 31] = 0.0; *halfcnt = 0; stageok[lane & 1] = 0; }
        d4 g;
#pragma unroll
        for (int t = 0; t < 4; t++) g[t] = Wc[16 * qa + lk + 4 * t][16 * qb + lr];
        d4 acc[2][2];
        zero_acc(acc);
        if (wv & 1) {
#pragma unroll
            for (int a = 0; a < 2; a++)
#pragma unroll
                for (int b = 0; b < 2; b++)
#pragma unroll
                    for (int t = 0; t < 4; t++) acc[a][b][t] = Wc[ro + 16 * a + lk + 4 * t][32 + 16 * b + lr];
        }
        d4 X2[2];
        double fb[8], dr[4][4];
        if (!first) {
#pragma unroll
            for (int u = 0; u < 8; u++) fb[u] = Lr[4 * u + lk][16 * wv + lr];
#pragma unroll
            for (int a = 0; a < 2; a++)
#pragma unroll
                for (int t = 0; t < 4; t++) X2[a][t] = Lr[32 + 16 * a + lk + 4 * t][16 * wv + lr];
#pragma unroll
            for (int q = 0; q < 4; q++)
#pragma unroll
                for (int t = 0; t < 4; t++) dr[q][t] = kp.rD[16 * q + lk + 4 * t];
        }
        __syncthreads();
        if (!first) {
            d4 W1[2] = { (d4){0, 0, 0, 0}, (d4){0, 0, 0, 0} }, W2[2] = { (d4){0, 0, 0, 0}, (d4){0, 0, 0, 0} };
            const int sw = 16 * (lk & 1);
#pragma unroll
            for (int u = 0; u < 8; u++) {
                const double* rowp = &kp.T1[(4 * u + lk) * 33];
                if (u < 4) W1[0] = __builtin_amdgcn_mfma_f64_16x16x4f64(rowp[lr], fb[u], W1[0], 0, 0, 0);
                W1[1] = __builtin_amdgcn_mfma_f64_16x16x4f64(rowp[16 + lr], fb[u], W1[1], 0, 0, 0);
            }
#pragma unroll
            for (int u = 0; u < 8; u++) {
                const double* rowp = &kp.Ep[(4 * u + lk) * 32];
                X2[0] = __builtin_amdgcn_mfma_f64_16x16x4f64(-rowp[lr ^ sw], W1[u >> 2][u & 3], X2[0], 0, 0, 0);
                X2[1] = __builtin_amdgcn_mfma_f64_16x16x4f64(-rowp[(16 + lr) ^ sw], W1[u >> 2][u & 3], X2[1], 0, 0, 0);
            }
#pragma unroll
            for (int u = 0; u < 8; u++) {
                const double* rowp = &kp.T2[(4 * u + lk) * 33];
                if (u < 4) W2[0] = __builtin_amdgcn_mfma_f64_16x16x4f64(rowp[lr], X2[u >> 2][u & 3], W2[0], 0, 0, 0);
                W2[1] = __builtin_amdgcn_mfma_f64_16x16x4f64(rowp[16 + lr], X2[u >> 2][u & 3], W2[1], 0, 0, 0);
            }
#pragma unroll
            for (int a = 0; a < 2; a++)
#pragma unroll
                for (int t = 0; t < 4; t++) {
                    const int jj = 16 * a + lk + 4 * t, cc = 16 * wv + lr;
                    Wc[jj][cc] = W1[a][t];       Lr[jj][cc] = W1[a][t] * dr[a][t];
                    Wc[32 + jj][cc] = W2[a][t];  Lr[32 + jj][cc] = W2[a][t] * dr[2 + a][t];
                }
        }
        if (wv0) GMW_TS(sy, p, 1);
        __syncthreads();
        if (!first) {
#pragma unroll
            for (int k = 0; k < 64; k += 4)
                g = __builtin_amdgcn_mfma_f64_16x16x4f64(-Lr[k + lk][16 * qa + lr], Wc[k + lk][16 * qb + lr], g, 0, 0, 0);
        }
#pragma unroll
        for (int t = 0; t < 4; t++) ws.Xm[16 * qa + lk + 4 * t][16 * qb + lr] = g[t];
        __syncthreads();
        if (wv0) GMW_TS(sy, p, 2);
        if (wv0) { gmw_cols_pivot_wave(ws, eps, lane); GMW_TS(sy, p + 64, 4); }
        else if (wvu == 2) { gmw_cols_t_wave<0>(ws, lane, nullptr, kp.T1); GMW_TS(sy, p + 64, 5); }
        else {
            if (!first) {
#pragma unroll
                for (int k = 0; k < 64; k += 4) {
                    const double a0 = -Lr[k + lk][ro + lr], a1 = -Lr[k + lk][ro + 16 + lr];
                    const double b0 = Wc[k + lk][32 + lr], b1 = Wc[k + lk][48 + lr];
                    acc[0][0] = __builtin_amdgcn_mfma_f64_16x16x4f64(a0, b0, acc[0][0], 0, 0, 0);
                    acc[0][1] = __builtin_amdgcn_mfma_f64_16x16x4f64(a0, b1, acc[0][1], 0, 0, 0);
                    acc[1][0] = __builtin_amdgcn_mfma_f64_16x16x4f64(a1, b0, acc[1][0], 0, 0, 0);
                    acc[1][1] = __builtin_amdgcn_mfma_f64_16x16x4f64(a1, b1, acc[1][1], 0, 0, 0);
                }
            }
            double (*X)[32] = (wv == 1) ? X01 : X11;
#pragma unroll
            for (int a = 0; a < 2; a++)
#pragma unroll
                for (int b = 0; b < 2; b++)
#pragma unroll
                    for (int t = 0; t < 4; t++) X[16 * a + lk + 4 * t][16 * b + lr] = acc[a][b][t];
            if (!first) {
                const int c4 = lr * 4;
#pragma unroll 4
                for (int i = 0; i < 8; i++) {
                    const int row = ro + 4 * i + lk;
                    const double sq = kp.sq[row];
                    d4 w = *(const d4*)&Wc[row][c4];
                    w[0] *= sq; w[1] *= sq; w[2] *= sq; w[3] *= sq;
                    *(d4*)&Sout[(size_t)(j0 + row) * ld + base + c4] = w;
                }
            }
            if (wv1) GMW_TS(sy, p + 64, 6); else GMW_TS(sy, p + 64, 7);
        }
        __syncthreads();
        if (wv0) GMW_TS(sy, p, 3);
        {
            d4 wq = (d4){0, 0, 0, 0};
#pragma unroll
            for (int u = 0; u < 8; u++)
                wq = __builtin_amdgcn_mfma_f64_16x16x4f64(kp.T1[(4 * u + lk) * 33 + 16 * qa + lr], X01[4 * u + lk][16 * qb + lr], wq, 0, 0, 0);
#pragma unroll
            for (int t = 0; t < 4; t++) {
                const int k = 16 * qa + lk + 4 * t, cc = 16 * qb + lr;
                const double e = wq[t] * gmw_pivot_rcp(ws.Dv[k]);
                Wc[k][cc] = wq[t];
                Lr[k][cc] = e;
                kp.Ep[k * 32 + (cc ^ (16 * (k & 1)))] = e;
            }
        }
        __syncthreads();
        if (!half_only) {
            d4 x;
#pragma unroll
            for (int t = 0; t < 4; t++) x[t] = X11[16 * qa + lk + 4 * t][16 * qb + lr];
#pragma unroll
            for (int k = 0; k < 32; k += 4)
                x = __builtin_amdgcn_mfma_f64_16x16x4f64(-Lr[k + lk][16 * qa + lr], Wc[k + lk][16 * qb + lr], x, 0, 0, 0);
#pragma unroll
            for (int t = 0; t < 4; t++) ws2.Xm[16 * qa + lk + 4 * t][16 * qb + lr] = x[t];
        }
        __syncthreads();
        if (wv0) GMW_TS(sy, p, 4);
        unsigned long long early = 0;
        if (wv0) { if (!half_only) gmw_cols_pivot_wave(ws2, eps, lane); GMW_TS(sy, p + 64, 0); }
        else if (wvu == 2) {
            if (!half_only) {
            unsigned long long fa = 0, fb = 0;
            if (p >= 1 && p + 1 < Tp) {
                fa = __hip_atomic_load(&ver[GMW_VIDX(p, p + 1, T)], __ATOMIC_RELAXED, __HIP_MEMORY_SCOPE_AGENT);
                fb = __hip_atomic_load(&ver[GMW_VIDX((p + 1), p + 1, T)], __ATOMIC_RELAXED, __HIP_MEMORY_SCOPE_AGENT);
            }
            gmw_cols_t_wave<2>(ws2, lane, nxt->Tt2, kp.T2, [&] {
                if (p == 0 || gmw_uniform64(fa) >= ebase + p) stageok[0] = 1;
                if (p == 0 || gmw_uniform64(fb) >= ebase + p) stageok[1] = 1;
            });
            GMW_TS(sy, p + 192, 0);
            }
        } else {
            const int c4 = (lane & 7) * 4;
            if (wv1) {
#pragma unroll
                for (int i = 0; i < 4; i++) {
                    const int row = 8 * i + (lane >> 3);
                    st_d4<true>(&nxt->E[row * 32 + c4], *(const d4*)&Lr[row][c4]);
                }
                if (lane < 32) {
                    const double D = ws.Dv[lane], rc = gmw_pivot_rcp(D), sq = sqrt(D) * rc;
                    st_dev(&nxt->D[lane], D); st_dev(&nxt->sq[lane], sq); st_dev(&nxt->rD[lane], rc);
                }
            } else gmw_copy_t<true>(kp.T1, nxt->Tt1, lane);
            asm volatile("s_waitcnt vmcnt(0)" ::: "memory");
            {
                int prev = 0;
                if (lane == 0) prev = __hip_atomic_fetch_add(halfcnt, 1, __ATOMIC_RELAXED, __HIP_MEMORY_SCOPE_WORKGROUP);
                if (__builtin_amdgcn_readfirstlane(prev) == 1) gmw_set_panel_flag(sy->half_ready, ebase + p + 1, lane);
            }
            if (!wv1) {
#pragma unroll
                for (int i = 0; i < 4; i++) {
                    const int row = 8 * i + (lane >> 3);
                    const double Dr = ws.Dv[row];
                    const double sq = (base + row < n) ? sqrt(Dr) * gmw_pivot_rcp(Dr) : 0.0;
                    d4 w = *(const d4*)&Wc[row][c4];
                    w[0] *= sq; w[1] *= sq; w[2] *= sq; w[3] *= sq;
                    *(d4*)&Sout[(size_t)(base + row) * ld + base + 32 + c4] = w;
                }
            }
            gmw_cols_out_wave<true>(ws, wv1 ? 0 : 1, lane, n, ld, base, nxt->D, nxt->sq, nxt->rD, Dall, Sout, kp.sq, kp.rD);
            if (!half_only) gmw_cols_out_wave<true>(ws2, wv1 ? 0 : 1, lane, n, ld, base + 32, nxt->D + 32, nxt->sq + 32, nxt->rD + 32, Dall, Sout, kp.sq + 32, kp.rD + 32,
                                                    [&] { if (p >= 1 && p + 1 < Tp) early = __hip_atomic_load(&ver[GMW_VIDX((wv1 ? p : p + 1), p + 1, T)], __ATOMIC_RELAXED, __HIP_MEMORY_SCOPE_AGENT); });
            if (wv1) GMW_TS(sy, p + 64, 1); else GMW_TS(sy, p + 64, 2);
        }
        if (p + 1 < Tp) {
            const bool tileA = wvu < 2;
            const int tr = tileA ? p : p + 1, r0 = (wvu & 1) ? 0 : 32;
            if (wv1) GMW_TS(sy, p, 5);
            const bool ready = p == 0 || gmw_uniform64(early) >= ebase + p || __builtin_amdgcn_readfirstlane(stageok[tileA ? 0 : 1]) != 0 ||
                               gmw_wait_ge(&ver[GMW_VIDX(tr, p + 1, T)], ebase + p, &sy->abort);
            if (wv1) GMW_TS(sy, p, 6);
            if (!ready) *okp = 0;
            else {
                double (*dst)[G64_LS] = tileA ? Lr : Wc;
                const double* src = G + (size_t)(64 * tr + r0) * ld + 64 * (p + 1) + lane;
                double v[32];
#pragma unroll
                for (int r = 0; r < 32; r++) v[r] = ld_dev(src + (size_t)r * ld);
#pragma unroll
                for (int r = 0; r < 32; r++) dst[r0 + r][lane] = v[r];
            }
        }
        else asm volatile("s_waitcnt vmcnt(0)" ::: "memory");
        __syncthreads();
        if (wv3 && p + 1 < T) { gmw_set_panel_flag(sy->panel_ready, ebase + p + 1, lane); GMW_TS(sy, p + 64, 3); }
        if (wv0) GMW_TS(sy, p, 7);
        if (!*okp) { if (wv0) gmw_abandon(sy, 1); return; }
    }
}

#ifndef GMW_MEM_EARLY2
#define GMW_MEM_EARLY2 0
#endif
struct GmwOwned { int I, J, nsteps; bool computed; int kfirst; bool passon; };
struct KDimsLite { int n, ld; };
__device__ __forceinline__ bool gmw_owner_step(int n, int ld, int T, int k, const GmwOwned& tl, d4 (&acc)[2][2], double* __restrict__ G,
                                               GmwPanel64* pans, double* __restrict__ Sout, GmwSync* sy, unsigned long long ebase,
                                               double (*Lr)[G64_LS], double (*Wc)[G64_LS], int* okp, bool wv0, int tid, bool memtile = false, bool rows32 = false)
{
    unsigned long long* ver = gmw_sync_ver(sy);
    if (wv0) {
        const unsigned long long want = ebase + k;
        unsigned long long a = want, b = want, pr = 0;
        for (int spins = 0; spins < GMW_XWG_LIMIT; spins++) {
            if (k > 0) {
                a = __hip_atomic_load(&ver[GMW_VIDX(k, tl.I, T)], __ATOMIC_RELAXED, __HIP_MEMORY_SCOPE_AGENT);
                b = __hip_atomic_load(&ver[GMW_VIDX(k, tl.J, T)], __ATOMIC_RELAXED, __HIP_MEMORY_SCOPE_AGENT);
            }
            pr = __hip_atomic_load(&sy->panel_ready[(blockIdx.x % GMW_FLAG_COPIES) * GMW_FLAG_STRIDE], __ATOMIC_RELAXED, __HIP_MEMORY_SCOPE_AGENT);
            a = gmw_uniform64(a); b = gmw_uniform64(b); pr = gmw_uniform64(pr);
            if (a >= want && b >= want) break;
            if ((spins & 31) == 31 && __builtin_amdgcn_readfirstlane(__hip_atomic_load(&sy->abort, __ATOMIC_RELAXED, __HIP_MEMORY_SCOPE_AGENT))) break;
            __builtin_amdgcn_s_sleep(1);
        }
        *okp = (a >= want && b >= want) ? ((pr >= ebase + k + 1) ? 2 : 1) : 0;
    }
    __syncthreads();
    if (!*okp) return false;
    const bool behind = *okp == 2;
    const bool last = k == tl.nsteps - 1;
    __syncthreads();
    return gmw_tile_update<true>(n, ld, 64 * k, tl.I - k - 1, tl.J - k - 1, G, pans + k, Sout, Lr, Wc, tid, acc, !tl.passon && (memtile || (k == 0 && !tl.computed)),
                                 !tl.passon && (memtile || last),
        [&] {
            if (!behind) { if (wv0) *okp = gmw_wait_ge(&sy->half_ready[(blockIdx.x % GMW_FLAG_COPIES) * GMW_FLAG_STRIDE], ebase + k + 1, &sy->abort); }
            __syncthreads();
            return *okp != 0;
        },
        [&] {
            if (!behind) { if (wv0) *okp = gmw_wait_ge(&sy->panel_ready[(blockIdx.x % GMW_FLAG_COPIES) * GMW_FLAG_STRIDE], ebase + k + 1, &sy->abort); }
            __syncthreads();
            return *okp != 0;
        },
        [&] { if (last && !tl.passon) gmw_publish(&ver[GMW_VIDX(tl.I, tl.J, T)], ebase + tl.nsteps, wv0); },
        behind && (!memtile || GMW_MEM_EARLY2 > 0), rows32 && tl.passon, memtile && GMW_MEM_EARLY2 == 1);
}

#define GMW_OWNED_MAX 2
#define GMW_OWNED_MEM 6
struct GmwTile { short I, J, nsteps, pad; };
#define GMW_HEAD_ROWS 2
#define GMW_HEAD_EXTRA_DIAG 2
__device__ __forceinline__ bool gmw_owner_computes(int I, int J) { return I >= GMW_HEAD_ROWS && !(I < GMW_HEAD_ROWS + GMW_HEAD_EXTRA_DIAG && J < GMW_HEAD_ROWS + GMW_HEAD_EXTRA_DIAG); }
template <bool DEEP = true>
__device__ __forceinline__ void gmw_owner_syrk(const KDimsLite d, const double* __restrict__ S0, const double* __restrict__ Ut0, int u0, int u1,
                                               int I, int J, d4 (&acc)[2][2], FrameScalars* __restrict__ fs, int tid, int krows)
{
    const int lane = tid & 63, wv = tid >> 6, lr = lane & 15, lk = lane >> 4;
    const int m0 = 64 * I + 32 * (wv >> 1), c0 = 64 * J + 32 * (wv & 1);
    zero_acc(acc);
    if (m0 >= d.ld || c0 >= d.ld || c0 + 32 <= m0) return;
    if constexpr (DEEP) {
        tile32_tn_deep<false>(acc, S0, d.ld, S0, d.ld, m0, c0, 0, min(m0 + 32, krows), lane);
        tile32_tn_deep<true>(acc, Ut0, d.ld, Ut0, d.ld, m0, c0, u0, u1, lane);
    } else {
        tile32_tn<false>(acc, S0, d.ld, S0, d.ld, m0, c0, 0, min(m0 + 32, krows), lane);
        tile32_tn<true>(acc, Ut0, d.ld, Ut0, d.ld, m0, c0, u0, u1, lane);
    }
    double gmax = 0.0, xmax = 0.0;
#pragma unroll
    for (int a = 0; a < 2; a++)
#pragma unroll
        for (int b = 0; b < 2; b++)
#pragma unroll
            for (int t = 0; t < 4; t++) {
                const int r = m0 + 16 * a + lk + 4 * t, c = c0 + 16 * b + lr;
                if (r < d.n && c < d.n && c >= r) { if (r == c) gmax = fmax(gmax, acc[a][b][t]); else xmax = fmax(xmax, acc[a][b][t]); }
            }
    gmax = wave_max(gmax); xmax = wave_max(xmax);
    if (lane == 0) {
        if (gmax > 0.0) atomicMax(&fs->gmax_bits, (unsigned long long)__double_as_longlong(gmax));
        if (xmax > 0.0) atomicMax(&fs->ximax_bits, (unsigned long long)__double_as_longlong(xmax));
    }
}

template <bool DEEP>
__device__ __forceinline__ void syrk_own_body(int n, int ld, const double* __restrict__ S0, const double* __restrict__ Ut0, int u0, int u1, int krows,
                                              double* __restrict__ G, FrameScalars* __restrict__ fs, const GmwTile* __restrict__ tiles, int nreal, const int bid)
{
    const GmwTile t = tiles[nreal - 1 - bid];
    if (!gmw_owner_computes(t.I, t.J)) return;
    const int tid = threadIdx.x, lane = tid & 63, wv = tid >> 6, lr = lane & 15, lk = lane >> 4;
    d4 acc[2][2];
    const KDimsLite dl = { n, ld };
    gmw_owner_syrk<DEEP>(dl, S0, Ut0, u0, u1, t.I, t.J, acc, fs, tid, krows);
    const int m0 = 64 * t.I + 32 * (wv >> 1), c0 = 64 * t.J + 32 * (wv & 1);
    if (m0 >= ld || c0 >= ld || c0 + 32 <= m0) return;
#pragma unroll
    for (int a = 0; a < 2; a++)
#pragma unroll
        for (int b = 0; b < 2; b++)
#pragma unroll
            for (int tt = 0; tt < 4; tt++) G[(size_t)(m0 + 16 * a + lk + 4 * tt) * ld + c0 + 16 * b + lr] = acc[a][b][tt];
}
__global__ __launch_bounds__(256) void k_syrk_own(int n, int ld, const double* __restrict__ S0, const double* __restrict__ Ut0, int u0, int u1, int krows,
                                                  double* __restrict__ G, FrameScalars* __restrict__ fs, const GmwTile* __restrict__ tiles, int nreal)
{
    syrk_own_body<true>(n, ld, S0, Ut0, u0, u1, krows, G, fs, tiles, nreal, (int)blockIdx.x);
}
__global__ __launch_bounds__(256) __attribute__((amdgpu_waves_per_eu(4, 8))) void k_syrk_own_b(int n, int ld, const SyrkOwnArgs* __restrict__ tab, int B, int u0, int u1, int krows, const GmwTile* __restrict__ tiles, int nreal)
{
    const int f = (int)blockIdx.x % B, bid = (int)blockIdx.x / B;
    const SyrkOwnArgs a = tab[f];
    syrk_own_body<false>(n, ld, a.S0, a.Ut0, u0, u1, krows, a.G, a.fs, tiles, nreal, bid);
}

__device__ int g_gmw_admitted = 0;
__global__ void k_gmw_gate(FrameScalars* __restrict__ fs, int limit)
{
    if (fs->frozen) return;
    if (threadIdx.x != 0) return;
    for (int spins = 0; spins < (1 << 22); spins++) {
        const int cur = __hip_atomic_load(&g_gmw_admitted, __ATOMIC_RELAXED, __HIP_MEMORY_SCOPE_AGENT);
        if (cur < limit && atomicCAS(&g_gmw_admitted, cur, cur + 1) == cur) return;
        __builtin_amdgcn_s_sleep(8);
    }
    atomicAdd(&g_gmw_admitted, 1);
    atomicAdd(&fs->gate_timeouts, 1);
}

__device__ __forceinline__ void gmw_head_tile_job(int n, int ld, int krows, const double* __restrict__ S0, const double* __restrict__ Ut0, int u0, int u1,
                                                  int2 tl, double* __restrict__ G, FrameScalars* __restrict__ fs, double* smem, int tid, GmwSync* sy = nullptr, bool stamp = false)
{
    if (tl.x < 0) return;
    double (*red)[64][17] = (double (*)[64][17])smem;
    const int lane = tid & 63, wv = tid >> 6, lr = lane & 15, lk = lane >> 4;
    const int m0 = tl.x * 32, n0 = tl.y * 32;
    d4 acc[2][2];
    zero_acc(acc);
    const int ke = min(m0 + 32, krows);
    const int ngs = ke >> 4, ngu = (u1 - u0) >> 4, ng = ngs + ngu;
    const int g0 = (ng * wv) >> 2, g1 = (ng * (wv + 1)) >> 2;
    if (g0 < ngs) tile32_tn_deep<false>(acc, S0, ld, S0, ld, m0, n0, g0 << 4, min(g1, ngs) << 4, lane);
    if (stamp && wv == 0) GMW_TS(sy, 132, 1);
    if (g1 > ngs) tile32_tn_deep<true>(acc, Ut0, ld, Ut0, ld, m0, n0, u0 + ((max(g0, ngs) - ngs) << 4), u0 + ((g1 - ngs) << 4), lane);
    if (stamp && wv == 0) GMW_TS(sy, 132, 2);
    if (stamp && wv == 3) GMW_TS(sy, 132, 6);
    splitk_reduce(acc, red, wv, lane);
    if (stamp && wv == 0) GMW_TS(sy, 132, 3);
    if (wv != 0) return;
    double gmax = 0.0, xmax = 0.0;
#pragma unroll
    for (int a = 0; a < 2; a++)
#pragma unroll
        for (int b = 0; b < 2; b++)
#pragma unroll
            for (int t = 0; t < 4; t++) {
                const int r = m0 + 16 * a + lk + 4 * t, c = n0 + 16 * b + lr;
                const double v = acc[a][b][t];
                st_dev(&G[(size_t)r * ld + c], v);
                if (r < n && c < n) { if (r == c) gmax = fmax(gmax, v); else xmax = fmax(xmax, v); }
            }
    gmax = wave_max(gmax); xmax = wave_max(xmax);
    if (lane == 0) {
        if (gmax > 0.0) atomicMax(&fs->gmax_bits, (unsigned long long)__double_as_longlong(gmax));
        if (xmax > 0.0) atomicMax(&fs->ximax_bits, (unsigned long long)__double_as_longlong(xmax));
    }
}
__device__ __forceinline__ bool gmw_wait_head(const unsigned int* cnt, unsigned int want, const int* abort_flag)
{
    for (int spins = 0; spins < GMW_XWG_LIMIT; spins++) {
        if ((unsigned)__builtin_amdgcn_readfirstlane((int)__hip_atomic_load(cnt, __ATOMIC_RELAXED, __HIP_MEMORY_SCOPE_AGENT)) >= want) return true;
        if ((spins & 31) == 31 && __builtin_amdgcn_readfirstlane(__hip_atomic_load(abort_flag, __ATOMIC_RELAXED, __HIP_MEMORY_SCOPE_AGENT))) return false;
        __builtin_amdgcn_s_sleep(1);
    }
    return false;
}

template <bool MEM>
__global__ __launch_bounds__(256) void k_gmw_persist(int n, int ld, int T, int Tp, double* __restrict__ G, GmwPanel64* __restrict__ pans,
                                                     double* __restrict__ Sout, double* __restrict__ Dall, double eps,
                                                     GmwSync* __restrict__ sy, const GmwTile* __restrict__ tiles, int ntiles,
                                                     FrameScalars* __restrict__ fs,
                                                     const double* __restrict__ S0, const double* __restrict__ Ut0, int u0, int u1, int krows, int gated,
                                                     const HeadArgs ha)
{
    __shared__ double Lr[64][G64_LS];
    __shared__ double Wc[64][G64_LS];
    __shared__ double facreg[2 * GMW_FAC_DOUBLES];
    __shared__ double xreg[1024 + 1024 + 32 * 33];
    __shared__ double keepreg[1024 + 64 + 64];
    __shared__ int ok, halfcnt, stageok[2];
    const int tid = threadIdx.x;
    const int nhelp = ha.nhelp;
    const int nmain = (int)gridDim.x - nhelp;
    const int role = (int)blockIdx.x < nmain ? (int)blockIdx.x : -1;
    int2 mytile = make_int2(-1, -1);
    unsigned long long t01 = 0, t23 = 0, t45 = 0;
    const int npass = (!MEM && Tp < T) ? T - Tp : 0, nreal = ntiles - npass;
    if (!MEM) {
        if (role < 0) { const int hb = (int)blockIdx.x - nmain; if (hb < ha.ntiles) mytile = ha.tiles[hb]; }
        else if (role > 0) {
            const unsigned long long* tq = (const unsigned long long*)tiles;
            if (role - 1 < nreal) t01 = tq[role - 1];
            if (role - 1 + nmain - 1 < nreal) t23 = tq[role - 1 + nmain - 1];
            if (role - 1 < npass) t45 = tq[nreal + role - 1];
        }
    }
    int frozen_now = fs->frozen;
    unsigned long long epoch_now = sy->epoch;
    if constexpr (MEM) asm volatile("" : "+s"(frozen_now), "+s"(epoch_now));
    else asm volatile("" : "+v"(mytile.x), "+v"(mytile.y), "+v"(t01), "+v"(t23), "+v"(t45), "+v"(frozen_now), "+v"(epoch_now));
    if (frozen_now) return;
    const unsigned long long ebase = epoch_now << GMW_EPOCH_SHIFT;
    if (role < 0) {
        if constexpr (!MEM) {
        const int nhead = ha.ntiles + ha.ndx + ha.ngd;
        const int wvu = __builtin_amdgcn_readfirstlane(tid >> 6), lane = tid & 63;
        const int job = (int)blockIdx.x - nmain;
#ifdef SRUKF_GMW_DBG
        if (tid == 0) atomicAdd(&sy->pad[1], 1ull);
#endif
        if ((int)blockIdx.x == nmain) GMW_TS(sy, 131, 0);
        if (job < ha.ntiles) {
            if (job == 0) GMW_TS(sy, 132, 0);
            gmw_head_tile_job(n, ld, krows, S0, Ut0, u0, u1, mytile, G, fs, &Lr[0][0], tid, sy, job == 0);
            if (job == 0) GMW_TS(sy, 132, 4);
            asm volatile("s_waitcnt vmcnt(0)" ::: "memory");
            __syncthreads();
            if (job == 0) GMW_TS(sy, 132, 5);
            if (job < ha.ncrit && job < 32) GMW_TS(sy, 140 + job, 0);
            if (wvu == 0) { if (lane == 0) __hip_atomic_fetch_add(job < ha.ncrit ? gmw_head_crit(sy) : gmw_head_done(sy), 1u, __ATOMIC_RELAXED, __HIP_MEMORY_SCOPE_AGENT); }
        } else if (job < ha.ntiles + ha.ndx) {
            const int dj = job - ha.ntiles;
            if (ha.ra.prep_next && dj == 0 && tid == 255) fs->ctl_next_valid = srukf_prepare_control(fs, fs->frame + 1) ? 1 : 0;
            srukf_gain_dx_job(n, ld, ha.dxp, ha.X, dj, ha.xr1, ha.ra.f32round, ha.ra.dxN);
        } else if (job < nhead) srukf_rank_gdiag_job(n, ld, u1, ha.ra, &fs->gmax_bits, job - ha.ntiles - ha.ndx);
        if ((int)blockIdx.x == nmain) GMW_TS(sy, 131, 1);
        if ((int)blockIdx.x == (int)gridDim.x - 1) GMW_TS(sy, 131, 2);
#ifdef SRUKF_GMW_DBG
        __syncthreads();
        if (tid == 0) atomicAdd(&sy->pad[2], 1ull);
#endif
        }
    } else if (role == 0) {
        bool head_ok = true;
        GMW_TS(sy, 128, 0);
        if (ha.ntiles > 0) {
            if (__builtin_amdgcn_readfirstlane(tid >> 6) == 0) ok = gmw_wait_head(gmw_head_crit(sy), (unsigned)ha.ncrit, &sy->abort) ? 1 : 0;
            __syncthreads();
            head_ok = ok != 0;
            __syncthreads();
        }
        GMW_TS(sy, 128, 1);
        if (head_ok) gmw_pivot_persist(n, ld, T, Tp, eps, G, pans, Dall, Sout, sy, ebase, Lr, Wc, facreg, xreg, keepreg, &ok, &halfcnt, stageok, tid, krows);
        else if (__builtin_amdgcn_readfirstlane(tid >> 6) == 0) gmw_abandon(sy, 2);
        GMW_TS(sy, 128, 2);
    } else {
        const bool wv0 = __builtin_amdgcn_readfirstlane(tid >> 6) == 0;
        const int workers = nmain - 1, w = role - 1;
        bool good = true;
        const bool half_last = (Tp < T) && (krows <= 64 * (Tp - 1) + 32);
        if constexpr (MEM) {
            int kmax = 0;
            for (int m = 0; m < GMW_OWNED_MEM; m++) if (w + m * workers < ntiles) kmax = max(kmax, (int)tiles[w + m * workers].nsteps);
            for (int k = 0; k < kmax && good; k++)
                for (int m = 0; m < GMW_OWNED_MEM && good; m++) {
                    const int ti = w + m * workers;
                    if (ti >= ntiles) break;
                    const GmwTile t = tiles[ti];
                    if (k >= t.nsteps) continue;
                    if (k < t.pad) continue;
                    const GmwOwned tm = { t.I, t.J, t.nsteps, false, t.pad, Tp < T && t.I == Tp };
                    d4 accm[2][2];
                    zero_acc(accm);
                    good = gmw_owner_step(n, ld, T, k, tm, accm, G, pans, Sout, sy, ebase, Lr, Wc, &ok, wv0, tid, true, half_last && k == Tp - 1);
                }
        } else {
        GmwOwned ta = { 0, 0, 0, false, 0, false }, tb = { 0, 0, 0, false, 0, false }, tc = { 0, 0, 0, false, 0, false };
        auto entry = [](unsigned long long q) { GmwTile t; t.I = (short)(q & 0xffff); t.J = (short)((q >> 16) & 0xffff); t.nsteps = (short)((q >> 32) & 0xffff); t.pad = (short)((q >> 48) & 0xffff); return t; };
        if (w < nreal) { const GmwTile t = entry(t01); ta.I = t.I; ta.J = t.J; ta.nsteps = t.nsteps; ta.kfirst = t.pad; ta.passon = Tp < T && t.I == Tp; }
        if (w + workers < nreal) { const GmwTile t = entry(t23); tb.I = t.I; tb.J = t.J; tb.nsteps = t.nsteps; tb.kfirst = t.pad; tb.passon = Tp < T && t.I == Tp; }
        if (w < npass) { const GmwTile t = entry(t45); tc.I = t.I; tc.J = t.J; tc.nsteps = t.nsteps; tc.kfirst = t.pad; tc.passon = true; tc.computed = true; }
        d4 acca[2][2], accb[2][2];
        zero_acc(acca); zero_acc(accb);
        if (role == 1) GMW_TS(sy, 129, 0);
        if (role == nmain - 1) GMW_TS(sy, 130, 0);
        if (S0) {
            const KDimsLite dl = { n, ld };
            if (ta.nsteps > 0 && gmw_owner_computes(ta.I, ta.J)) { if (!ta.passon) gmw_owner_syrk(dl, S0, Ut0, u0, u1, ta.I, ta.J, acca, fs, tid, krows); ta.computed = true; }
            if (tb.nsteps > 0 && gmw_owner_computes(tb.I, tb.J)) { if (!tb.passon) gmw_owner_syrk(dl, S0, Ut0, u0, u1, tb.I, tb.J, accb, fs, tid, krows); tb.computed = true; }
        }
        if (role == 1) GMW_TS(sy, 129, 1);
        if (role == nmain - 1) GMW_TS(sy, 130, 1);
        if (ha.ntiles > 0) {
            if (wv0) ok = (gmw_wait_head(gmw_head_crit(sy), (unsigned)ha.ncrit, &sy->abort) && gmw_wait_head(gmw_head_done(sy), (unsigned)(ha.ntiles - ha.ncrit), &sy->abort)) ? 1 : 0;
            __syncthreads();
            good = ok != 0;
            if (!good && wv0) gmw_abandon(sy, 3);
            __syncthreads();
        }
        if (role == 1) GMW_TS(sy, 129, 2);
        if (role == nmain - 1) GMW_TS(sy, 130, 2);
        const int kmax = max(ta.nsteps, tb.nsteps);
        for (int k = 0; k < kmax && good; k++) {
            if (k < ta.nsteps && k >= ta.kfirst) good = gmw_owner_step(n, ld, T, k, ta, acca, G, pans, Sout, sy, ebase, Lr, Wc, &ok, wv0, tid, false, half_last && k == Tp - 1);
            if (good && k < tb.nsteps && k >= tb.kfirst) good = gmw_owner_step(n, ld, T, k, tb, accb, G, pans, Sout, sy, ebase, Lr, Wc, &ok, wv0, tid, false, half_last && k == Tp - 1);
        }
        if (good && tc.nsteps > 0) good = gmw_owner_step(n, ld, T, tc.kfirst, tc, acca, G, pans, Sout, sy, ebase, Lr, Wc, &ok, wv0, tid, false, half_last);
        }
        if (!good && wv0) gmw_abandon(sy, 4);
        if (role == 1) GMW_TS(sy, 129, 3);
        if (role == nmain - 1) GMW_TS(sy, 130, 3);
    }
    GMW_DBG(sy, 6, 7777);
    __syncthreads();
    if (tid == 0) {
        const unsigned int done = __hip_atomic_fetch_add(&sy->exited, 1u, __ATOMIC_RELAXED, __HIP_MEMORY_SCOPE_AGENT);
        if (done == gridDim.x - 1) {
            if (__hip_atomic_load(&sy->abort, __ATOMIC_RELAXED, __HIP_MEMORY_SCOPE_AGENT)) { atomicAdd(&fs->clamp_rows, 1); atomicMin(&fs->clamp_first, 0); atomicAdd(&fs->gmw_aborts, 1); }
#ifdef SRUKF_GMW_DBG
            sy->pad[3] = __hip_atomic_load(gmw_head_done(sy), __ATOMIC_RELAXED, __HIP_MEMORY_SCOPE_AGENT); sy->pad[4] = __hip_atomic_load(gmw_head_crit(sy), __ATOMIC_RELAXED, __HIP_MEMORY_SCOPE_AGENT);
            sy->pad[5] = gridDim.x; sy->pad[6] = (unsigned long long)nhelp;
#endif
            __hip_atomic_store(&sy->abort, 0, __ATOMIC_RELAXED, __HIP_MEMORY_SCOPE_AGENT);
            __hip_atomic_store(&sy->exited, 0u, __ATOMIC_RELAXED, __HIP_MEMORY_SCOPE_AGENT);
            __hip_atomic_store(gmw_head_done(sy), 0u, __ATOMIC_RELAXED, __HIP_MEMORY_SCOPE_AGENT);
            __hip_atomic_store(gmw_head_crit(sy), 0u, __ATOMIC_RELAXED, __HIP_MEMORY_SCOPE_AGENT);
            __hip_atomic_store(&sy->resident, 0u, __ATOMIC_RELAXED, __HIP_MEMORY_SCOPE_AGENT);
            __hip_atomic_store(&sy->epoch, (ebase >> GMW_EPOCH_SHIFT) + 1, __ATOMIC_RELAXED, __HIP_MEMORY_SCOPE_AGENT);
            if (gated) atomicSub(&g_gmw_admitted, 1);
        }
    }
}

__global__ __launch_bounds__(256) void k_gmw_pivslab_persist(int n, int ld, int T, int Tp, double* __restrict__ G, GmwPanel64* __restrict__ pans,
                                                             double* __restrict__ Sout, double* __restrict__ Dall, double eps, GmwSync* __restrict__ sy,
                                                             FrameScalars* __restrict__ fs, int krows, double* __restrict__ Wslab, double* __restrict__ Lslab,
                                                             unsigned int total_exits)
{
    __shared__ double Lr[64][G64_LS];
    __shared__ double Wc[64][G64_LS];
    __shared__ double facreg[2 * GMW_FAC_DOUBLES];
    __shared__ double xreg[1024 + 1024 + 32 * 33];
    __shared__ double keepreg[1024 + 64 + 64];
    __shared__ int ok, halfcnt, stageok[2];
    const int tid = threadIdx.x, lane = tid & 63;
    int frozen_now = fs->frozen;
    unsigned long long epoch_now = sy->epoch;
    asm volatile("" : "+s"(frozen_now), "+s"(epoch_now));
    if (frozen_now) return;
    const unsigned long long ebase = epoch_now << GMW_EPOCH_SHIFT;
    if (tid == 0) __hip_atomic_fetch_add(&sy->resident, 1u, __ATOMIC_RELAXED, __HIP_MEMORY_SCOPE_AGENT);
    const bool wv0 = __builtin_amdgcn_readfirstlane(tid >> 6) == 0;
    if (blockIdx.x == 0) {
        gmw_pivot_persist(n, ld, T, Tp, eps, G, pans, Dall, Sout, sy, ebase, Lr, Wc, facreg, xreg, keepreg, &ok, &halfcnt, stageok, tid, krows);
    } else {
        const int J = (int)blockIdx.x, wv = tid >> 6;
        unsigned long long* ver = gmw_sync_ver(sy);
        unsigned long long* slabver = gmw_sync_slabver(sy, T);
        const bool half_last = (Tp < T) && (krows <= 64 * (Tp - 1) + 32);
        const int kend = min(J, Tp);
        bool good = true;
        for (int k = 0; k < kend && good; k++) {
            if (wv0) {
                bool g2 = gmw_wait_ge(&sy->panel_ready[(blockIdx.x % GMW_FLAG_COPIES) * GMW_FLAG_STRIDE], ebase + k + 1, &sy->abort);
                if (g2 && k >= 1) g2 = gmw_wait_ge(&ver[GMW_VIDX(k, J, T)], ebase + k, &sy->abort);
                ok = g2 ? 1 : 0;
            }
            __syncthreads();
            good = ok != 0;
            if (good) {
                const bool r32 = half_last && k == Tp - 1;
                gmw_slab16_to_global<true>(n, ld, 64 * k, 64 * J + 16 * wv, G, pans + k, Sout, Wslab + (size_t)k * 64 * ld, Lslab + (size_t)k * 64 * ld, J >= k + 2 || (Tp < T && k == Tp - 1), r32, lane);
                gmw_publish(&slabver[GMW_VIDX(k, J, T)], ebase + 1, wv0);
            }
            __syncthreads();
        }
        if (!good && wv0) gmw_abandon(sy, 5);
    }
    __syncthreads();
    if (tid == 0) {
        const unsigned int done = __hip_atomic_fetch_add(&sy->exited, 1u, __ATOMIC_RELAXED, __HIP_MEMORY_SCOPE_AGENT);
        if (done == total_exits - 1) {
            if (__hip_atomic_load(&sy->abort, __ATOMIC_RELAXED, __HIP_MEMORY_SCOPE_AGENT)) { atomicAdd(&fs->clamp_rows, 1); atomicMin(&fs->clamp_first, 0); atomicAdd(&fs->gmw_aborts, 1); }
            __hip_atomic_store(&sy->abort, 0, __ATOMIC_RELAXED, __HIP_MEMORY_SCOPE_AGENT);
            __hip_atomic_store(&sy->exited, 0u, __ATOMIC_RELAXED, __HIP_MEMORY_SCOPE_AGENT);
            __hip_atomic_store(&sy->resident, 0u, __ATOMIC_RELAXED, __HIP_MEMORY_SCOPE_AGENT);
            __hip_atomic_store(&sy->epoch, (ebase >> GMW_EPOCH_SHIFT) + 1, __ATOMIC_RELAXED, __HIP_MEMORY_SCOPE_AGENT);
        }
    }
}
__global__ __launch_bounds__(256) __attribute__((amdgpu_waves_per_eu(4, 8)))
void k_gmw_tiles_persist(int ld, int T, double* __restrict__ G, GmwSync* __restrict__ sy, const GmwTile* __restrict__ tiles, FrameScalars* __restrict__ fs,
                         const double* __restrict__ Wslab, const double* __restrict__ Lslab, unsigned int total_exits)
{
    __shared__ int ok;
    const int tid = threadIdx.x, lane = tid & 63, wv = tid >> 6, lr = lane & 15, lk = lane >> 4;
    const unsigned long long tq = ((const unsigned long long*)tiles)[blockIdx.x];
    int frozen_now = fs->frozen;
    unsigned long long epoch_now = sy->epoch;
    if (frozen_now) return;
    const unsigned long long ebase = epoch_now << GMW_EPOCH_SHIFT;
    const int I = (int)(short)(tq & 0xffff), J = (int)(short)((tq >> 16) & 0xffff), ns = (int)(short)((tq >> 32) & 0xffff);
    const bool wv0 = __builtin_amdgcn_readfirstlane(wv) == 0;
    unsigned long long* ver = gmw_sync_ver(sy);
    const unsigned long long* slabver = gmw_sync_slabver(sy, T);
    const int m0 = 64 * I + 32 * (wv >> 1), c0 = 64 * J + 32 * (wv & 1);
    const bool live = (m0 < ld) && (c0 < ld) && (c0 + 32 > m0);
    d4 acc[2][2];
    zero_acc(acc);
    if (live) {
#pragma unroll
        for (int a = 0; a < 2; a++)
#pragma unroll
            for (int b = 0; b < 2; b++)
#pragma unroll
                for (int t = 0; t < 4; t++) acc[a][b][t] = G[(size_t)(m0 + 16 * a + lk + 4 * t) * ld + c0 + 16 * b + lr];
    }
    bool good = true;
    for (int k = 0; k < ns && good; k++) {
        if (wv0) {
            const unsigned long long want = ebase + 1;
            unsigned long long a = 0, b = 0;
            for (int spins = 0; spins < GMW_XWG_LIMIT; spins++) {
                a = gmw_uniform64(__hip_atomic_load(&slabver[GMW_VIDX(k, I, T)], __ATOMIC_RELAXED, __HIP_MEMORY_SCOPE_AGENT));
                b = gmw_uniform64(__hip_atomic_load(&slabver[GMW_VIDX(k, J, T)], __ATOMIC_RELAXED, __HIP_MEMORY_SCOPE_AGENT));
                if (a >= want && b >= want) break;
                if ((spins & 31) == 31 && __builtin_amdgcn_readfirstlane(__hip_atomic_load(&sy->abort, __ATOMIC_RELAXED, __HIP_MEMORY_SCOPE_AGENT))) break;
                if (I - k <= 2) __builtin_amdgcn_s_sleep(2); else __builtin_amdgcn_s_sleep(32);
            }
            ok = (a >= want && b >= want) ? 1 : 0;
        }
        __syncthreads();
        good = ok != 0;
        if (good && live) {
            const double* __restrict__ Lb = Lslab + (size_t)k * 64 * ld + m0 + lr;
            const double* __restrict__ Wb = Wslab + (size_t)k * 64 * ld + c0 + lr;
#pragma unroll
            for (int kk = 0; kk < 64; kk += 16) {
                double a0[4], a1[4], b0[4], b1[4];
#pragma unroll
                for (int u = 0; u < 4; u++) {
                    const size_t ro = (size_t)(kk + 4 * u + lk) * ld;
                    a0[u] = Lb[ro]; a1[u] = Lb[ro + 16]; b0[u] = Wb[ro]; b1[u] = Wb[ro + 16];
                }
#pragma unroll
                for (int u = 0; u < 4; u++) {
                    acc[0][0] = __builtin_amdgcn_mfma_f64_16x16x4f64(-a0[u], b0[u], acc[0][0], 0, 0, 0);
                    acc[0][1] = __builtin_amdgcn_mfma_f64_16x16x4f64(-a0[u], b1[u], acc[0][1], 0, 0, 0);
                    acc[1][0] = __builtin_amdgcn_mfma_f64_16x16x4f64(-a1[u], b0[u], acc[1][0], 0, 0, 0);
                    acc[1][1] = __builtin_amdgcn_mfma_f64_16x16x4f64(-a1[u], b1[u], acc[1][1], 0, 0, 0);
                }
            }
        }
        __syncthreads();
    }
    if (good) {
        if (live) {
#pragma unroll
            for (int a = 0; a < 2; a++)
#pragma unroll
                for (int b = 0; b < 2; b++)
#pragma unroll
                    for (int t = 0; t < 4; t++) st_dev(&G[(size_t)(m0 + 16 * a + lk + 4 * t) * ld + c0 + 16 * b + lr], acc[a][b][t]);
        }
        gmw_publish(&ver[GMW_VIDX(I, J, T)], ebase + ns, wv0);
    } else if (wv0) gmw_abandon(sy, 6);
    __syncthreads();
    if (tid == 0) {
        const unsigned int done = __hip_atomic_fetch_add(&sy->exited, 1u, __ATOMIC_RELAXED, __HIP_MEMORY_SCOPE_AGENT);
        if (done == total_exits - 1) {
            if (__hip_atomic_load(&sy->abort, __ATOMIC_RELAXED, __HIP_MEMORY_SCOPE_AGENT)) { atomicAdd(&fs->clamp_rows, 1); atomicMin(&fs->clamp_first, 0); atomicAdd(&fs->gmw_aborts, 1); }
            __hip_atomic_store(&sy->abort, 0, __ATOMIC_RELAXED, __HIP_MEMORY_SCOPE_AGENT);
            __hip_atomic_store(&sy->exited, 0u, __ATOMIC_RELAXED, __HIP_MEMORY_SCOPE_AGENT);
            __hip_atomic_store(&sy->resident, 0u, __ATOMIC_RELAXED, __HIP_MEMORY_SCOPE_AGENT);
            __hip_atomic_store(&sy->epoch, (ebase >> GMW_EPOCH_SHIFT) + 1, __ATOMIC_RELAXED, __HIP_MEMORY_SCOPE_AGENT);
        }
    }
}
__device__ __forceinline__ void gmw_form_job(int n, int ld, int krows, const double* __restrict__ A, const double* __restrict__ Ut, int mp, int tr, int tc,
// ... 323 lines not shown
```

cv-monoslam_amd/csrc/srukf_rank.h:

```cpp
#pragma once
#include <hip/hip_runtime.h>
#include "srukf_device.h"

struct RankArgs {
    double* A;
    double* Utp;
    double* gdiag;
    const int* iperm;
    const int* perm;
    int r;
    int dzperm;
    int f32round;
    int prep_next;
    int dxN;
};

struct Pxy2Args { const double* DZp; const double* A; double* P0; double* P1; MeasArgs ms; };
struct SyrkArgs { const double* S; const double* Ut; double* G; FrameScalars* fs; const double* dxp; double* X; RankArgs ra; const double* xr1; };
struct GainArgs {
    double* Ut; const double* PxyR; const double* Si; const int* vis; const double* h; const double* z_seq; const int* m_seq; FrameScalars* fs; double* dxp;
    RankArgs ra; const double* Cm; double* S; const double* P1; const double* DZp; const double* sigR; const double* Z0;
};
struct ExpandArgs {
    const double* Sp; const double* D; const int* perm; const int* iperm; const double* gdiag; FrameScalars* fs; const double* X; double* S; double* A;
    double* sigR; double* Z; double* DZ;
};

struct HeadArgs {
    const int2* tiles; int ntiles;
    int ncrit;
    const double* dxp; double* X; const double* xr1; int ndx;
    int ngd;
    int nhelp;
    RankArgs ra;
};

#define SRUKF_RANK_COLS 16
__device__ __forceinline__ double srukf_rank_colsq(const double* __restrict__ M, int ld, int rows, int a, int kl)
{
    double v = 0.0;
    for (int k = kl; k < rows; k += 20 * 16) {
        double t[20];
#pragma unroll
        for (int u = 0; u < 20; u++) t[u] = M[(size_t)min(k + 16 * u, rows - 1) * ld + a];
#pragma unroll
        for (int u = 0; u < 20; u++) v += (k + 16 * u < rows) ? t[u] * t[u] : 0.0;
    }
    return v;
}
__device__ __forceinline__ void srukf_rank_gdiag_job(int n, int ld, int mu, const RankArgs ra, unsigned long long* gmax_bits, int blk)
{
    __shared__ double cs[16][17];
    const int a = ra.r + SRUKF_RANK_COLS * blk + (threadIdx.x & 15), kl = threadIdx.x >> 4;
    double v = 0.0;
    if (a < n) v = srukf_rank_colsq(ra.A, ld, ra.r, a, kl) - srukf_rank_colsq(ra.Utp, ld, mu, a, kl);
    cs[kl][threadIdx.x & 15] = v;
    __syncthreads();
    if (threadIdx.x < 16 && a < n) {
        double t = 0.0;
        for (int q = 0; q < 16; q++) t += cs[q][threadIdx.x];
        ra.gdiag[a] = t;
        if (t > 0.0) atomicMax(gmax_bits, (unsigned long long)__double_as_longlong(t));
    }
}
```

cv-monoslam_amd/csrc/srukf_replay.hip:

```cpp

#include "srukf_ctx.h"
using namespace srukf_impl;

__global__ void k_refactor_reset(int np, unsigned long long* theta_bits, FrameScalars* fs, int reset_stats)
{
    const int i = blockIdx.x * blockDim.x + threadIdx.x;
    if (i < np) theta_bits[i] = 0ull;
    if (i == 0 && reset_stats) { fs->gmax_bits = 0ull; fs->ximax_bits = 0ull; }
}

__global__ void k_set_seq(FrameScalars* fs, const double* odo_seq, int seqF, double a1, double a2, double a3, double a4)
{
    fs->odo_seq = odo_seq; fs->seqF = seqF;
    fs->a[0] = a1; fs->a[1] = a2; fs->a[2] = a3; fs->a[3] = a4;
}

__global__ void k_set_frame(FrameScalars* fs, int frame, int clear_clamp)
{
    fs->frame = frame;
    srukf_prepare_control(fs);
    fs->stat_count = 0;
    fs->const_rows_ok = 0; fs->const_rows_pending = 0;
    for (int q = 0; q < SRUKF_STAT_GROUPS; q++) fs->stat_cnt[q] = 0;
    fs->traj_base = nullptr;
// ... 148 lines not shown

const double* take_xr1(srukf_ctx* c)
{
    if (!c->xr1_pending) return nullptr;
    c->xr1_pending = false;
    return (const double*)((const char*)c->fs + offsetof(FrameScalars, Xr1));
}

void seq_predict_fused(srukf_ctx* c, int mode)
{
    const KDims& d = c->d;
    ProfScope ps(c, mode == 2 ? KC_PROJECT_TABLE : KC_PROJECT_MOTION, 2.0 * 60.0 * d.Na * d.N + 60.0 * d.L, 8.0 * ((double)d.n * d.n / 2 + 2.0 * d.L * 2 * d.N + (double)d.n * 2 * d.N + 8.0 * d.L + 8.0 * d.n));
    if (mode == 2) srukf_launch_project_table(c->stream, d, c->w, c->p, c->X, c->S, c->sigR, c->Cmat, c->Z, c->DZ, c->fs, rank_args(c, false, c->dbg.pxy2 != 0), null_skip(c));
    else srukf_launch_project_motion(c->stream, d, c->w, c->p, c->X, c->S, c->sigR, c->Cmat, c->Z, c->DZ, c->fs, rank_args(c));
    c->xr1_pending = true;
}

void seq_predict_motion(srukf_ctx* c, const double* odo_pair_dev)
{
    const KDims& d = c->d;
    ProfScope ps(c, KC_MOTION, 60.0 * d.L, 8.0 * (4.0 * d.n + 8.0 * d.L + 4.0 * d.n));
    srukf_launch_motion(c->stream, d, c->w, c->p, c->X, c->S, c->sigR, c->Cmat, c->fs, c->odo_seq, odo_pair_dev, rank_args(c));
}

void seq_predict_measurement(srukf_ctx* c, bool fused_stats)
{
    const KDims& d = c->d;
    {
        ProfScope ps(c, KC_PROJECT, 2.0 * 60.0 * d.Na * d.N, 8.0 * ((double)d.n * d.n / 2 + 2.0 * d.L * 2 * d.N + (double)d.n * 2 * d.N));
        srukf_launch_project(c->stream, d, c->w, c->p, c->X, c->S, c->sigR, c->Z, c->DZ, c->fs);
    }
    if (!fused_stats) {
        ProfScope ps(c, KC_STATS, 30.0 * d.L * d.N, 8.0 * 3.0 * d.L * 2 * d.N);
        srukf_launch_meas_stats(c->stream, d, c->w, c->X, c->sigR, c->Z, c->mpart, c->h, c->Si, c->vis, c->PxyR);
    }
}

int gmw_fused_mode() { return g_dbg_gmw_fused; }

int rank_fused_mode() { return g_dbg_rank_fused; }

int rank_fold_mode() { return g_dbg_rank_fold; }

void shadow_rebuild(srukf_ctx* c)
{
    if (c->red_r > 0 && c->shadowA) srukf_launch_rank_shadow(c->stream, c->d.n, c->d.np, c->red_r, c->S, c->red_perm, c->shadowA);
}

bool gmw_plan_persists(const srukf_ctx* c, const GmwPlan& gp) { return gp.workers >= 0 || split_form(c, gp, true); }

bool gmw_use_persist(const srukf_ctx* c) { return gmw_persist_mode() && c->gmw_shared != 2 && gmw_plan_persists(c, c->gplan); }

}


namespace srukf_impl {

int plan_tenants(const srukf_ctx* c) { return c->gmw_shared == 1 ? c->shared_tenants : 1; }

int gate_limit(const srukf_ctx* c) { return c->gmw_shared == 1 ? c->shared_tenants : 0; }

void rank_expand(srukf_ctx* c, bool frame_tail, bool table, bool fuse)
{
    const int n = c->d.n, np = c->d.np;
    const bool f32s = c->storage != SRUKF_STORAGE_F64;
    const bool f32fuse = storage_f32_like(c) && fuse && table && frame_tail;
    const bool f32 = f32s && !f32fuse;
    const bool tt = table && frame_tail && !f32;
    const bool exports = c->step_export.dst && tt && fuse;
    srukf_launch_rank_expand(c->stream, n, np, c->red_r, c->p.epsilon, c->G, c->D, c->red_perm, c->red_iperm, c->gdiag, c->fs, c->X, (frame_tail && !f32) ? 1 : 0, c->S, c->shadowA,
                             tt ? c->sigR : nullptr, c->w.gamma, (tt && fuse) ? 1 : 0, c->d, c->w, c->p, c->Z, c->DZ, f32fuse ? 1 : 0, exports ? &c->step_export : nullptr,
                             c->storage == SRUKF_STORAGE_F32_MIXED ? 1e-6 * c->dbg.mixed_null_ppm : 0.0,
                             (tt && fuse) ? c->fold_sync : nullptr, c->fold_sync ? 4 * (c->d.mp / 64) * (c->d.np / 64) : 0);
    c->step_export_attached = exports;
    if (f32) {
        quantize_state(c);
        srukf_launch_rank_round(c->stream, np, c->red_r, c->shadowA);
        if (frame_tail) srukf_launch_traj(c->stream, c->d, c->X, c->S, c->fs, nullptr, 1);
    }
}

}

static int fold_tiles_pct(const srukf_ctx* c) { return c->gmw_shared == 1 ? 200 : 106; }

namespace srukf_impl {

bool replay_red_fused(const srukf_ctx* c)
{
    return c->red_r > 0 && c->storage != SRUKF_STORAGE_F32_MIXED && c->shadowA && c->w.wc0 == c->w.wm0 && gmw_use_persist(c) &&
           c->gplan_red.workers >= 0 && c->gplan_red.nreal <= c->gplan_red.workers * fold_tiles_pct(c) / 100 && c->gplan_red.T >= 16 &&
           !c->debug_starve && gmw_fused_mode() && rank_fused_mode() && rank_fold_mode();
}

bool replay_red_perm(const srukf_ctx* c)
{
    return c->red_r > 0 && (c->storage != SRUKF_STORAGE_F32_MIXED || (c->dbg.mixed_rank && c->A32)) && c->shadowA && c->w.wc0 == c->w.wm0 && rank_fused_mode() && c->dbg.table_perm;
}

int replay_motion_mode(const srukf_ctx* c)
{
    const bool st_ok = c->storage == SRUKF_STORAGE_F64 ||
                       (storage_f32_like(c) && c->dbg.f32_fuse && c->dbg.tail_fuse && c->dbg.pxy2 && c->dbg.nullskip && c->nskip && c->tail_ok &&
                        (size_t)c->d.np * sizeof(double) <= 48 * 1024);
    if (c->dbg.fused_motion == 2 && !((replay_red_fused(c) || replay_red_perm(c)) && st_ok && c->null_canonical)) return 1;
    return c->dbg.fused_motion;
}

bool replay_fuse_mode(const srukf_ctx* c)
{
    return replay_motion_mode(c) == 2 && c->dbg.pxy2 && c->dbg.nullskip && c->nskip && c->tail_ok && c->dbg.tail_fuse &&
           (size_t)c->d.np * sizeof(double) <= 48 * 1024;
}

}

#define SRUKF_HEAD_FOLD_MIN_FREE_CUS 32

namespace srukf_impl {

bool head_fold_ok(const srukf_ctx* c)
{
    const int need = g_dbg_head_fold_free.load() > 0 ? g_dbg_head_fold_free.load() : SRUKF_HEAD_FOLD_MIN_FREE_CUS;
    const int free_cus = c->gplan_red.cus - 1 - c->gplan_red.workers;
    const int nhelp = c->n_syrk_head_tiles + (c->d.n + 255) / 256 + (c->d.n - c->red_r + SRUKF_RANK_COLS - 1) / SRUKF_RANK_COLS;
    const bool pays = g_dbg_head_fold_free.load() > 0 || 4 * nhelp <= 9 * free_cus;
    return c->dbg.head_fold && c->gmw_shared == 0 && free_cus >= need && pays;
}

void seq_refactor(srukf_ctx* c, int ub, int ue, bool slow, bool keep_backup, bool need_reset, bool frame_tail, bool table, bool fuse)
{
    const KDims& d = c->d;
    const int np = d.np, n = d.n;
    if (need_reset || slow) {
        ProfScope ps(c, KC_MISC, 0, 8.0 * np);
        hipLaunchKernelGGL(k_refactor_reset, dim3((np + 255) / 256), dim3(256), 0, c->stream, np, c->theta, c->fs, 1);
    }
    const bool reduced = !slow && c->red_r > 0 && (c->storage != SRUKF_STORAGE_F32_MIXED || (c->dbg.mixed_rank && c->A32));
    const bool red_fused = reduced && !keep_backup && ub == 0 && ue == d.mp && replay_red_fused(c);
    if (red_fused) {
        const double rr = c->red_r, hr = srukf_gmw_head_rows();
        const double head_flop = 2.0 * hr * n * (hr / 2.0 + d.mp) + 2.0 * (n - rr) * (rr + d.mp), head_byte = 8.0 * ((hr + d.mp) * n + (n - rr) * (rr + d.mp));
        const bool head_fold = head_fold_ok(c);
        if (!head_fold) {
            ProfScope ps(c, KC_SYRK, head_flop, head_byte);
            srukf_launch_syrk(c->stream, d, c->shadowA, c->Utp, 0, d.mp, c->Wf, c->fs, c->syrk_head_tiles, c->n_syrk_head_tiles, dx_src(c), c->X, rank_args(c, table, false, fuse && storage_f32_like(c)), take_xr1(c));
            c->dx_pending = false;
        }
        {
            ProfScope ps(c, KC_GMW_PERSIST, c->red_fac_flop + c->red_own_flop + (head_fold ? head_flop : 0.0), 8.0 * (2.0 * rr * n + (double)d.mp * n));
            HeadArgs ha = {};
            if (head_fold) {
                ha.tiles = (const int2*)c->syrk_head_tiles; ha.ntiles = c->n_syrk_head_tiles; ha.ncrit = c->n_syrk_head_crit;
                ha.dxp = dx_src(c); ha.X = c->X; ha.xr1 = take_xr1(c); ha.ndx = c->dx_pending ? (n + 255) / 256 : 0;
                ha.ra = rank_args(c, table, false, fuse && storage_f32_like(c)); ha.ngd = (n - c->red_r + SRUKF_RANK_COLS - 1) / SRUKF_RANK_COLS;
                ha.nhelp = ha.ntiles + ha.ndx + ha.ngd;
                c->dx_pending = false;
            }
            srukf_launch_gmw_persist_head(c->stream, n, np, c->p.epsilon, c->Wf, c->gplan_red.pans, c->D, c->G, c->gplan_red.sync, c->gplan_red.tiles, c->gplan_red.ntiles,
                                          c->gplan_red.workers, c->fs, c->shadowA, c->Utp, 0, d.mp, c->red_Tp, (c->red_r + 15) & ~15, gate_limit(c), head_fold ? &ha : nullptr);
        }
        ProfScope ps(c, KC_RANK_EXPAND, 0, 8.0 * 2.5 * (double)n * n);
        rank_expand(c, frame_tail, table, fuse);
        return;
    }
    const bool red_perm = reduced && !red_fused && !keep_backup && ub == 0 && ue == d.mp && c->shadowA && c->w.wc0 == c->w.wm0 && rank_fused_mode();
    if (red_perm) {
        const double rr = c->red_r, rp = 64.0 * c->red_Tp;
        const bool own_order = c->gmw_shared == 1 && gmw_use_persist(c) && c->gplan_red.workers > 0 && c->gplan_red.T >= 16 && !c->debug_starve && gmw_fused_mode() && rank_fold_mode() &&
                               srukf_gmw_register_form(c->gplan_red.T, c->gplan_red.Tp, c->gplan_red.ntiles, c->gplan_red.workers);
        const bool sfold = !own_order && split_fold_ok(c);
        const double syrk_flop_all = rr * rr * rr / 3.0 + rr * rr * (n - rr) + 2.0 * d.mp * (rr * n - rr * rr / 2.0) + 2.0 * (n - rr) * (rr + d.mp);
        {
            ProfScope ps(c, KC_SYRK, sfold ? c->red_head0_flop + 2.0 * (n - rr) * (rr + d.mp) : syrk_flop_all, 8.0 * (rr * n + (double)d.mp * n + rp * n));
            if (c->storage == SRUKF_STORAGE_F32_MIXED) {
                if (c->dbg.mixed_bf16 && c->mxr_xt) {
                    srukf_launch_split_bf3(c->stream, c->mxr_krows, np, c->mxr_ktot, 0, c->shadowA, c->mxr_xt, c->mxr_xt_stride);
                    srukf_launch_split_bf3(c->stream, d.mp, np, c->mxr_ktot, c->mxr_krows, c->Utp, c->mxr_xt, c->mxr_xt_stride);
                    srukf_launch_syrk_bf3(c->stream, n, np, d.mp, c->mxr_krows, c->mxr_ktot, c->mxr_xt, c->mxr_xt_stride, c->mxr_tasks, c->mxr_ntasks, c->mxr_tiles, c->mxr_ntiles,
                                          c->mxr_part, c->Wf, c->fs);
                } else {
                    srukf_launch_cvt_f32(c->stream, (size_t)c->mxr_krows * np, c->shadowA, c->A32);
                    srukf_launch_cvt_f32(c->stream, (size_t)d.mp * np, c->Utp, c->U32);
                    srukf_launch_syrk32(c->stream, n, np, d.mp, c->A32, c->U32, c->mxr_tasks, c->mxr_ntasks, c->mxr_tiles, c->mxr_ntiles, c->mxr_part, c->Wf, c->fs, c->mxr_krows);
                }
                srukf_launch_syrk(c->stream, d, c->shadowA, c->Utp, 0, d.mp, c->Wf, c->fs, c->mxr_f64_tiles, c->dbg.mixed_f64_robot ? c->mxr_n_f64_tiles : 0,
                                  dx_src(c), c->X, rank_args(c, table, false, fuse && storage_f32_like(c)), take_xr1(c));
            } else if (own_order) {
                srukf_launch_syrk(c->stream, d, c->shadowA, c->Utp, 0, d.mp, c->Wf, c->fs, c->syrk_head_tiles, c->n_syrk_head_tiles, dx_src(c), c->X, rank_args(c, table, false, fuse && storage_f32_like(c)), take_xr1(c));
                srukf_launch_syrk_own(c->stream, n, np, c->shadowA, c->Utp, 0, d.mp, (c->red_r + 15) & ~15, c->Wf, c->fs, c->gplan_red.tiles, c->gplan_red.ntiles, c->red_Tp);
            } else if (sfold && c->dbg.split_fold != 2)
                srukf_launch_syrk(c->stream, d, c->shadowA, c->Utp, 0, d.mp, c->Wf, c->fs, c->red_head0_tiles, c->n_red_head0_tiles, dx_src(c), c->X, rank_args(c, table, false, fuse && storage_f32_like(c)), take_xr1(c));
            else
            srukf_launch_syrk(c->stream, d, c->shadowA, c->Utp, 0, d.mp, c->Wf, c->fs, c->red_syrk_tiles, c->n_red_syrk_tiles, dx_src(c), c->X, rank_args(c, table, false, fuse && storage_f32_like(c)), take_xr1(c));
            c->dx_pending = false;
        }
        {
            ProfScope ps(c, gmw_use_persist(c) && gmw_plan_persists(c, c->gplan_red) ? KC_GMW_PERSIST : KC_GMW_TRAIL, c->red_fac_flop + (sfold ? syrk_flop_all - c->red_head0_flop : 0.0), 8.0 * 2.0 * rp * n);
            launch_gmw_fast(c, c->Wf, c->G, true, sfold);
        }
        ProfScope ps(c, KC_RANK_EXPAND, 0, 8.0 * 2.5 * (double)n * n);
        rank_expand(c, frame_tail, table, fuse);
        return;
    }
    const bool fused = !reduced && !slow && !keep_backup && gmw_use_persist(c) && ub == 0 && ue == d.mp && c->storage == SRUKF_STORAGE_F64 &&
                       c->gplan.ntiles <= c->gplan.workers && c->gplan.T >= 16 &&
                       !c->debug_starve && gmw_fused_mode();
    const double nn = n;
    const double syrk_flop = nn * nn * nn / 3.0 + nn * nn * (ue - ub), syrk_byte = 8.0 * (nn * nn + (double)(ue - ub) * nn);
    const double head_frac = fused ? fmin(1.0, 2.0 * srukf_gmw_head_rows() / nn) : 1.0;
    if (c->storage == SRUKF_STORAGE_F32_MIXED && ub == 0 && ue == d.mp && !(c->dbg.mixed_rank && c->A32)) {
        ProfScope ps(c, KC_SYRK, syrk_flop, 4.0 * (nn * nn + (double)(ue - ub) * nn) + 8.0 * nn * nn / 2);
        if (c->dx_pending) srukf_launch_gain_dx(c->stream, n, np, c->dxp, c->X, take_xr1(c));
        c->dx_pending = false;
        srukf_launch_cvt_f32(c->stream, (size_t)d.mp * np, c->Ut, c->U32);
        srukf_launch_cvt_robot_cols(c->stream, n, np, c->S, c->S32);
        srukf_launch_syrk32(c->stream, n, np, d.mp, c->S32, c->U32, c->mx_tasks, c->mx_ntasks, c->mx_tiles, c->mx_ntiles, c->mx_part, c->G, c->fs, np);
    } else {
        ProfScope ps(c, KC_SYRK, syrk_flop * head_frac, syrk_byte * head_frac);
        srukf_launch_syrk(c->stream, d, c->S, c->Ut, ub, ue, c->G, c->fs, fused ? c->syrk_head_tiles : c->syrk_tiles,
                          fused ? c->n_syrk_head_tiles : c->n_syrk_tiles, dx_src(c), c->X, RankArgs{}, take_xr1(c));
        c->dx_pending = false;
    }
    if (keep_backup) hipMemcpyAsync(c->Gbak, c->G, sizeof(double) * (size_t)np * np, hipMemcpyDeviceToDevice, c->stream);
    if (reduced) {
        {
            ProfScope ps(c, KC_MISC, 0, 16.0 * nn * nn);
            hipLaunchKernelGGL(k_sym_permute, dim3(np), dim3(256), 0, c->stream, n, np, c->G, np, c->Wf, c->red_perm);
            srukf_launch_rank_diag(c->stream, n, np, c->G, c->red_perm, c->gdiag);
        }
        {
            const double rr = 64.0 * c->red_Tp;
            ProfScope ps(c, gmw_use_persist(c) && gmw_plan_persists(c, c->gplan_red) ? KC_GMW_PERSIST : KC_GMW_TRAIL, rr * rr * rr / 3.0 + rr * rr * (nn - rr) + rr * (nn - rr) * (nn - rr) / 2.0,
                         8.0 * (rr * nn));
            launch_gmw_fast(c, c->Wf, c->G, true);
        }
        ProfScope ps(c, KC_GMW_CHECK, 0, 8.0 * nn * nn);
        rank_expand(c, frame_tail);
        return;
    }
    if (!slow) {
        auto panel_flop = [&](int j0) { const double r2 = np - j0 - 64; return j0 < 0 ? 64.0 * 64.0 * 64.0 / 3.0 : 64.0 * r2 * r2 + 3.0 * 2.0 * 32.0 * 32.0 * r2 + 64.0 * 64.0 * 64.0 / 3.0; };
        auto panel_byte = [&](int j0) { const double r2 = np - j0 - 64; return 8.0 * (r2 * r2 + 2.0 * 64.0 * r2); };
        if (gmw_use_persist(c)) {
            double fl = 0.0, by = 0.0;
            for (int j0 = -64; j0 + 64 < np; j0 += 64) { fl += panel_flop(j0); by += panel_byte(j0); }
            ProfScope ps(c, KC_GMW_PERSIST, fl + syrk_flop * (1.0 - head_frac), by + syrk_byte * (1.0 - head_frac));
            if (fused) srukf_launch_gmw_persist(c->stream, n, np, c->p.epsilon, c->G, c->gplan.pans, c->D, c->Wf, c->gplan.sync, c->gplan.tiles, c->gplan.ntiles,
                                                c->gplan.workers, c->fs, c->S, c->Ut, ub, ue, 0, 0, gate_limit(c));
            else launch_gmw_fast(c, c->G, c->S);
        } else {
            int pb = 0;
            for (int j0 = -64; j0 + 64 < np; j0 += 64, pb ^= 1) {
                ProfScope ps(c, KC_GMW_TRAIL, panel_flop(j0), panel_byte(j0));
                srukf_launch_gmw_step64(c->stream, n, np, j0, c->p.epsilon, c->G, c->pan[pb ^ 1], c->pan[pb], c->D, c->S, c->fs);
            }
        }
        quantize_state(c);
        ProfScope ps(c, KC_GMW_CHECK, 0, 8.0 * (double)n * n / 2);
        srukf_launch_gmw_check(c->stream, n, np, c->D, fused ? c->Wf : c->S, c->fs, c->X, frame_tail ? 1 : 0, fused ? c->S : nullptr);
    } else {
        ProfScope ps(c, KC_GMW_COL, (double)n * n * n / 3.0, 8.0 * (double)n * n * n / 3.0);
        exact_path(c, c->G, c->S);
        quantize_state(c);
        if (frame_tail) srukf_launch_traj(c->stream, d, c->X, c->S, c->fs, nullptr, 1);
    }
    shadow_rebuild(c);
}

bool split_fold_ok(const srukf_ctx* c)
{
    const GmwPlan& gp = c->gplan_red;
    const bool fits = gp.nreal <= 4 * (gp.cus - gp.T) || g_dbg_fold_force.load() != 0;
    return c->dbg.split_fold && (fits || c->dbg.split_fold == 2) && c->red_r > 0 && c->storage != SRUKF_STORAGE_F32_MIXED && c->split_fold_list && c->n_split_fold > 0 && c->red_head0_tiles &&
           !c->debug_starve && !c->dbg.split_record && gmw_use_persist(c) && gmw_plan_persists(c, gp) && split_form(c, gp, true);
}

void launch_gmw_fast(srukf_ctx* c, double* Gbuf, double* Sout, bool reduced, bool fold)
{
    const int np = c->d.np, n = c->d.n;
    const GmwPlan& gp = reduced ? c->gplan_red : c->gplan;
    const int Tp = reduced ? c->red_Tp : np / 64;
    if (gmw_use_persist(c) && gmw_plan_persists(c, gp)) {
        const int workers = c->debug_starve == 1 ? 0 : gp.workers;
        if (split_form(c, gp, true)) {
            if (c->dbg.split_record) hipMemcpyAsync(c->Gbak, Gbuf, sizeof(double) * (size_t)np * np, hipMemcpyDeviceToDevice, c->stream);
            hipEventRecord(c->ev_fork, c->stream);
            hipStreamWaitEvent(c->side, c->ev_fork, 0);
            if (fold && reduced) c->split_fold_seqs++;
            if (fold && reduced)
                srukf_launch_gmw_split_fold(c->stream, c->side, n, np, c->p.epsilon, Gbuf, gp.pans, c->D, Sout, gp.sync, c->split_fold_list, c->n_split_fold, c->fs, Tp, (c->red_r + 15) & ~15,
                                            c->gsW, c->gsL, c->shadowA, c->Utp, c->d.mp);
            else
            srukf_launch_gmw_split(c->stream, c->side, n, np, c->p.epsilon, Gbuf, gp.pans, c->D, Sout, gp.sync, gp.tiles, gp.ntiles, c->fs, Tp, reduced ? ((c->red_r + 15) & ~15) : 0, c->gsW, c->gsL, c->debug_starve ? 1 : 0);
            hipEventRecord(c->ev_join, c->side);
            hipStreamWaitEvent(c->stream, c->ev_join, 0);
            return;
        }
        srukf_launch_gmw_persist(c->stream, n, np, c->p.epsilon, Gbuf, gp.pans, c->D, Sout, gp.sync, gp.tiles, gp.ntiles, workers, c->fs, nullptr, nullptr, 0, 0, Tp,
                                 reduced ? ((c->red_r + 15) & ~15) : 0, gate_limit(c));
        return;
    }
    int pb = 0;
    for (int j0 = -64; j0 + 64 < np && j0 + 64 <= 64 * Tp; j0 += 64, pb ^= 1)
        srukf_launch_gmw_step64(c->stream, n, np, j0, c->p.epsilon, Gbuf, c->pan[pb ^ 1], c->pan[pb], c->D, Sout, c->fs);
}
// ... 580 lines not shown
```

Before: 5546 frames/s.

## Start GMW pivot after first 64x64 head tiles, gating later panels on remaining crit tiles

Reorders the head SYRK tile list so tiles in the first 64-row block come first, and counts them with a separate crit0 counter. The pivot worker now waits only on those tiles before starting panel 0, then waits on the rest of the critical tiles when staging panel 1. Head tile jobs also publish their completion counter before doing the gmax/xmax atomic reductions, moving those atomics off the critical path. The aim is to shorten the serial head latency before factorization begins. The cost is extra synchronization complexity and a new abort path.

```diff
diff --git a/cv-monoslam_amd/csrc/srukf_api.hip b/cv-monoslam_amd/csrc/srukf_api.hip
--- a/cv-monoslam_amd/csrc/srukf_api.hip
+++ b/cv-monoslam_amd/csrc/srukf_api.hip
@@ -273,19 +273,26 @@
         ALLOC(c->syrk_tiles, ts.size()); ALLOC(c->pxy_tiles, tp.size());
         std::vector<int> th;
         const int hd = srukf_gmw_head_rows(), hx = hd + 64 * srukf_gmw_head_extra_diag();
+        std::vector<int> th2;
         for (int pass = 0; pass < 2; pass++)
             for (size_t q = 0; q + 1 < ts.size(); q += 2) {
                 if (!(ts[q] >= 0 && (ts[q] * 32 < hd || (ts[q] * 32 < hx && ts[q + 1] * 32 < hx)))) continue;
                 const bool crit = ts[q] * 32 < 128 && ts[q + 1] * 32 < 128;
-                if (crit == (pass == 0)) { th.push_back(ts[q]); th.push_back(ts[q + 1]); }
+                if (crit == (pass == 0)) { th2.push_back(ts[q]); th2.push_back(ts[q + 1]); }
             }
-        c->n_syrk_head_crit = 0;
-        for (size_t q = 0; q + 1 < th.size(); q += 2) if (th[q] * 32 < 128 && th[q + 1] * 32 < 128) c->n_syrk_head_crit++;
+        c->n_syrk_head_crit = 0; c->n_syrk_head_crit0 = 0;
+        for (int pass = 0; pass < 2; pass++)
+            for (size_t q = 0; q + 1 < th2.size(); q += 2) {
+                const bool crit0 = th2[q] * 32 < 64 && th2[q + 1] * 32 < 64;
+                if (crit0 == (pass == 0)) { th.push_back(th2[q]); th.push_back(th2[q + 1]); }
+                if (pass == 0 && crit0) c->n_syrk_head_crit0++;
+                if (pass == 0 && th2[q] * 32 < 128 && th2[q + 1] * 32 < 128) c->n_syrk_head_crit++;
+            }
         c->n_syrk_head_tiles = (int)th.size() / 2;
         ALLOC(c->syrk_head_tiles, th.size() ? th.size() : 2);
         {
             std::vector<int> qx[8], tb;
-            for (size_t q = 0; q + 1 < th.size(); q += 2) { const int x = (th[q + 1] / 2) % 8; qx[x].push_back(th[q]); qx[x].push_back(th[q + 1]); }
+            for (size_t q = 0; q + 1 < th2.size(); q += 2) { const int x = (th2[q + 1] / 2) % 8; qx[x].push_back(th2[q]); qx[x].push_back(th2[q + 1]); }
             size_t longest = 0;
             for (int x = 0; x < 8; x++) longest = std::max(longest, qx[x].size() / 2);
             for (size_t rnd = 0; rnd < longest; rnd++)
diff --git a/cv-monoslam_amd/csrc/srukf_ctx.h b/cv-monoslam_amd/csrc/srukf_ctx.h
--- a/cv-monoslam_amd/csrc/srukf_ctx.h
+++ b/cv-monoslam_amd/csrc/srukf_ctx.h
@@ -175,6 +175,7 @@
         int table_perm = 1;
         int tail_fuse = 1;
         int head_fold = 1;
+        int head_start = 1;
         int nullskip = 1;
         int pxy2 = 1;
         int step_fuse_export = 1;
@@ -198,7 +199,7 @@
     double *ckS = nullptr, *ckX = nullptr;
     int *syrk_tiles = nullptr, *pxy_tiles = nullptr;
     int *syrk_head_tiles = nullptr;
-    int n_syrk_tiles = 0, n_pxy_tiles = 0, n_syrk_head_tiles = 0, n_syrk_head_crit = 0;
+    int n_syrk_tiles = 0, n_pxy_tiles = 0, n_syrk_head_tiles = 0, n_syrk_head_crit = 0, n_syrk_head_crit0 = 0;
     int* syrk_head_tiles_b = nullptr; int n_syrk_head_tiles_b = 0;
     FrameScalars* fs = nullptr;
     int seqF = 0;
diff --git a/cv-monoslam_amd/csrc/srukf_debug.hip b/cv-monoslam_amd/csrc/srukf_debug.hip
--- a/cv-monoslam_amd/csrc/srukf_debug.hip
+++ b/cv-monoslam_amd/csrc/srukf_debug.hip
@@ -96,6 +96,7 @@
     else if (!strcmp(key, "pxy2")) c->dbg.pxy2 = value ? 1 : 0;
     else if (!strcmp(key, "nullskip")) c->dbg.nullskip = value ? 1 : 0;
     else if (!strcmp(key, "head_fold")) c->dbg.head_fold = value ? 1 : 0;
+    else if (!strcmp(key, "head_start")) c->dbg.head_start = value ? 1 : 0;
     else if (!strcmp(key, "tail_fuse")) c->dbg.tail_fuse = value ? 1 : 0;
     else if (!strcmp(key, "table_perm")) c->dbg.table_perm = value ? 1 : 0;
     else if (!strcmp(key, "f32_fuse")) c->dbg.f32_fuse = value ? 1 : 0;
@@ -164,6 +165,7 @@
     else if (!strcmp(key, "step_fast")) *value = c->step_fast_frames;
     else if (!strcmp(key, "step_slow")) *value = c->step_slow_frames;
     else if (!strcmp(key, "exact_frames")) *value = c->exact_frames;
+    else if (!strcmp(key, "head_start")) *value = c->dbg.head_start;
     else if (!strcmp(key, "fold_seqs")) *value = c->fold_seqs;
     else if (!strcmp(key, "split_fold_seqs")) *value = c->split_fold_seqs;
     else if (!strncmp(key, "pxy2_stamp", 10) && key[10] >= '1' && key[10] <= '7') { const unsigned long long* t = (const unsigned long long*)(c->hmeas + c->d.mp + 5 * (size_t)c->d.N); *value = (long long)(t[key[10] - '0'] - t[0]); }
diff --git a/cv-monoslam_amd/csrc/srukf_device.h b/cv-monoslam_amd/csrc/srukf_device.h
--- a/cv-monoslam_amd/csrc/srukf_device.h
+++ b/cv-monoslam_amd/csrc/srukf_device.h
@@ -324,6 +324,7 @@
 };
 __device__ __forceinline__ unsigned int* gmw_head_crit(GmwSync* sy) { return (unsigned int*)&sy->panel_ready[GMW_FLAG_STRIDE / 2]; }
 __device__ __forceinline__ unsigned int* gmw_head_done(GmwSync* sy) { return (unsigned int*)&sy->half_ready[GMW_FLAG_STRIDE / 2]; }
+__device__ __forceinline__ unsigned int* gmw_head_crit0(GmwSync* sy) { return (unsigned int*)&sy->panel_ready[GMW_FLAG_STRIDE + GMW_FLAG_STRIDE / 2]; }
 __device__ __forceinline__ unsigned long long* gmw_sync_ver(GmwSync* sy) { return (unsigned long long*)(sy + 1); }
 #define GMW_VER_STRIDE 16
 #define GMW_VIDX(I, J, T) (((size_t)(I) * (T) + (J)) * GMW_VER_STRIDE)
diff --git a/cv-monoslam_amd/csrc/srukf_gmw_persist.hip b/cv-monoslam_amd/csrc/srukf_gmw_persist.hip
--- a/cv-monoslam_amd/csrc/srukf_gmw_persist.hip
+++ b/cv-monoslam_amd/csrc/srukf_gmw_persist.hip
@@ -27,6 +27,15 @@
     }
     return false;
 }
+__device__ __forceinline__ bool gmw_wait_head(const unsigned int* cnt, unsigned int want, const int* abort_flag)
+{
+    for (int spins = 0; spins < GMW_XWG_LIMIT; spins++) {
+        if ((unsigned)__builtin_amdgcn_readfirstlane((int)__hip_atomic_load(cnt, __ATOMIC_RELAXED, __HIP_MEMORY_SCOPE_AGENT)) >= want) return true;
+        if ((spins & 31) == 31 && __builtin_amdgcn_readfirstlane(__hip_atomic_load(abort_flag, __ATOMIC_RELAXED, __HIP_MEMORY_SCOPE_AGENT))) return false;
+        __builtin_amdgcn_s_sleep(1);
+    }
+    return false;
+}
 __device__ __forceinline__ void gmw_abandon(GmwSync* sy, unsigned int site)
 {
     __hip_atomic_store(&sy->abort, 1, __ATOMIC_RELAXED, __HIP_MEMORY_SCOPE_AGENT);
@@ -68,7 +77,8 @@
 __device__ __forceinline__ void gmw_pivot_persist(int n, int ld, int T, int Tp, double eps, double* __restrict__ G, GmwPanel64* __restrict__ pans,
                                                   double* __restrict__ Dall, double* __restrict__ Sout, GmwSync* sy, unsigned long long ebase,
                                                   double (*Lr)[G64_LS], double (*Wc)[G64_LS], double* facreg, double* xreg, double* keepreg,
-                                                  int* okp, int* halfcnt, int* stageok, int tid, int klim)
+                                                  int* okp, int* halfcnt, int* stageok, int tid, int klim,
+                                                  const unsigned int* crit1 = nullptr, unsigned int crit1_want = 0, bool stage4 = false)
 {
     const int lane = tid & 63, wv = tid >> 6, lr = lane & 15, lk = lane >> 4;
     const int qa = wv >> 1, qb = wv & 1;
@@ -82,7 +92,14 @@
     const int wvu = __builtin_amdgcn_readfirstlane(wv);
     const bool wv0 = wvu == 0, wv1 = wvu == 1, wv3 = wvu == 3;
     if (wv0) *okp = 1;
-    if (wv3) gmw_stage_tile(Wc, G, ld, 0, 0, lane);
+    if (stage4) {
+        const double* src = G + (size_t)(16 * wv) * ld + lane;
+        double v[16];
+#pragma unroll
+        for (int r = 0; r < 16; r++) v[r] = ld_dev(src + (size_t)r * ld);
+#pragma unroll
+        for (int r = 0; r < 16; r++) Wc[16 * wv + r][lane] = v[r];
+    } else if (wv3) gmw_stage_tile(Wc, G, ld, 0, 0, lane);
     __syncthreads();
     for (int p = 0; p < Tp; p++) {
         const int j0 = 64 * (p - 1), base = 64 * p;
@@ -228,13 +245,15 @@
         else if (wvu == 2) {
             if (!half_only) {
             unsigned long long fa = 0, fb = 0;
+            unsigned int fc = 0;
             if (p >= 1 && p + 1 < Tp) {
                 fa = __hip_atomic_load(&ver[GMW_VIDX(p, p + 1, T)], __ATOMIC_RELAXED, __HIP_MEMORY_SCOPE_AGENT);
                 fb = __hip_atomic_load(&ver[GMW_VIDX((p + 1), p + 1, T)], __ATOMIC_RELAXED, __HIP_MEMORY_SCOPE_AGENT);
-            }
+            } else if (p == 0 && crit1 && p + 1 < Tp) fc = __hip_atomic_load(crit1, __ATOMIC_RELAXED, __HIP_MEMORY_SCOPE_AGENT);
             gmw_cols_t_wave<2>(ws2, lane, nxt->Tt2, kp.T2, [&] {
-                if (p == 0 || gmw_uniform64(fa) >= ebase + p) stageok[0] = 1;
-                if (p == 0 || gmw_uniform64(fb) >= ebase + p) stageok[1] = 1;
+                const bool h0 = p == 0 && (!crit1 || (unsigned)__builtin_amdgcn_readfirstlane((int)fc) >= crit1_want);
+                if (h0 || (p > 0 && gmw_uniform64(fa) >= ebase + p)) stageok[0] = 1;
+                if (h0 || (p > 0 && gmw_uniform64(fb) >= ebase + p)) stageok[1] = 1;
             });
             GMW_TS(sy, p + 192, 0);
             }
@@ -277,8 +296,8 @@
             const bool tileA = wvu < 2;
             const int tr = tileA ? p : p + 1, r0 = (wvu & 1) ? 0 : 32;
             if (wv1) GMW_TS(sy, p, 5);
-            const bool ready = p == 0 || gmw_uniform64(early) >= ebase + p || __builtin_amdgcn_readfirstlane(stageok[tileA ? 0 : 1]) != 0 ||
-                               gmw_wait_ge(&ver[GMW_VIDX(tr, p + 1, T)], ebase + p, &sy->abort);
+            const bool ready = (p == 0 && !crit1) || (p > 0 && gmw_uniform64(early) >= ebase + p) || __builtin_amdgcn_readfirstlane(stageok[tileA ? 0 : 1]) != 0 ||
+                               (p == 0 ? gmw_wait_head(crit1, crit1_want, &sy->abort) : gmw_wait_ge(&ver[GMW_VIDX(tr, p + 1, T)], ebase + p, &sy->abort));
             if (wv1) GMW_TS(sy, p, 6);
             if (!ready) *okp = 0;
             else {
@@ -295,7 +314,7 @@
         __syncthreads();
         if (wv3 && p + 1 < T) { gmw_set_panel_flag(sy->panel_ready, ebase + p + 1, lane); GMW_TS(sy, p + 64, 3); }
         if (wv0) GMW_TS(sy, p, 7);
-        if (!*okp) { if (wv0) gmw_abandon(sy, 1); return; }
+        if (!*okp) { if (wv0) gmw_abandon(sy, (p == 0 && crit1) ? 8 : 1); return; }
     }
 }
 
@@ -430,7 +449,8 @@
 }
 
 __device__ __forceinline__ void gmw_head_tile_job(int n, int ld, int krows, const double* __restrict__ S0, const double* __restrict__ Ut0, int u0, int u1,
-                                                  int2 tl, double* __restrict__ G, FrameScalars* __restrict__ fs, double* smem, int tid, GmwSync* sy = nullptr, bool stamp = false)
+                                                  int2 tl, double* __restrict__ G, FrameScalars* __restrict__ fs, double* smem, int tid, double (&mx)[2], bool late,
+                                                  GmwSync* sy = nullptr, bool stamp = false)
 {
     if (tl.x < 0) return;
     double (*red)[64][17] = (double (*)[64][17])smem;
@@ -461,22 +481,21 @@
                 st_dev(&G[(size_t)r * ld + c], v);
                 if (r < n && c < n) { if (r == c) gmax = fmax(gmax, v); else xmax = fmax(xmax, v); }
             }
+    if (late) { mx[0] = gmax; mx[1] = xmax; return; }
     gmax = wave_max(gmax); xmax = wave_max(xmax);
     if (lane == 0) {
         if (gmax > 0.0) atomicMax(&fs->gmax_bits, (unsigned long long)__double_as_longlong(gmax));
         if (xmax > 0.0) atomicMax(&fs->ximax_bits, (unsigned long long)__double_as_longlong(xmax));
     }
 }
-__device__ __forceinline__ bool gmw_wait_head(const unsigned int* cnt, unsigned int want, const int* abort_flag)
-{
-    for (int spins = 0; spins < GMW_XWG_LIMIT; spins++) {
-        if ((unsigned)__builtin_amdgcn_readfirstlane((int)__hip_atomic_load(cnt, __ATOMIC_RELAXED, __HIP_MEMORY_SCOPE_AGENT)) >= want) return true;
-        if ((spins & 31) == 31 && __builtin_amdgcn_readfirstlane(__hip_atomic_load(abort_flag, __ATOMIC_RELAXED, __HIP_MEMORY_SCOPE_AGENT))) return false;
-        __builtin_amdgcn_s_sleep(1);
-    }
-    return false;
-}
-
+__device__ __forceinline__ void gmw_head_tile_stats_late(const double (&mx)[2], FrameScalars* __restrict__ fs, int lane)
+{
+    const double gmax = wave_max(mx[0]), xmax = wave_max(mx[1]);
+    if (lane == 0) {
+        if (gmax > 0.0) atomicMax(&fs->gmax_bits, (unsigned long long)__double_as_longlong(gmax));
+        if (xmax > 0.0) atomicMax(&fs->ximax_bits, (unsigned long long)__double_as_longlong(xmax));
+    }
+}
 template <bool MEM>
 __global__ __launch_bounds__(256) void k_gmw_persist(int n, int ld, int T, int Tp, double* __restrict__ G, GmwPanel64* __restrict__ pans,
                                                      double* __restrict__ Sout, double* __restrict__ Dall, double eps,
@@ -523,14 +542,21 @@
 #endif
         if ((int)blockIdx.x == nmain) GMW_TS(sy, 131, 0);
         if (job < ha.ntiles) {
-            if (job == 0) GMW_TS(sy, 132, 0);
-            gmw_head_tile_job(n, ld, krows, S0, Ut0, u0, u1, mytile, G, fs, &Lr[0][0], tid, sy, job == 0);
-            if (job == 0) GMW_TS(sy, 132, 4);
+            const bool stamped = job == ha.ncrit;
+            if (stamped) GMW_TS(sy, 132, 0);
+            const bool early = ha.start != 0;
+            double hmx[2] = { 0.0, 0.0 };
+            gmw_head_tile_job(n, ld, krows, S0, Ut0, u0, u1, mytile, G, fs, &Lr[0][0], tid, hmx, early, sy, stamped);
+            if (stamped) GMW_TS(sy, 132, 4);
             asm volatile("s_waitcnt vmcnt(0)" ::: "memory");
             __syncthreads();
-            if (job == 0) GMW_TS(sy, 132, 5);
+            if (stamped) GMW_TS(sy, 132, 5);
+            if (wvu == 0) {
+                unsigned int* cnt = job >= ha.ncrit ? gmw_head_done(sy) : (early && job < ha.ncrit0) ? gmw_head_crit0(sy) : gmw_head_crit(sy);
+                if (lane == 0) __hip_atomic_fetch_add(cnt, 1u, __ATOMIC_RELAXED, __HIP_MEMORY_SCOPE_AGENT);
+            }
             if (job < ha.ncrit && job < 32) GMW_TS(sy, 140 + job, 0);
-            if (wvu == 0) { if (lane == 0) __hip_atomic_fetch_add(job < ha.ncrit ? gmw_head_crit(sy) : gmw_head_done(sy), 1u, __ATOMIC_RELAXED, __HIP_MEMORY_SCOPE_AGENT); }
+            if (early && wvu == 0 && mytile.x >= 0) gmw_head_tile_stats_late(hmx, fs, lane);
         } else if (job < ha.ntiles + ha.ndx) {
             const int dj = job - ha.ntiles;
             if (ha.ra.prep_next && dj == 0 && tid == 255) fs->ctl_next_valid = srukf_prepare_control(fs, fs->frame + 1) ? 1 : 0;
@@ -547,13 +573,15 @@
         bool head_ok = true;
         GMW_TS(sy, 128, 0);
         if (ha.ntiles > 0) {
-            if (__builtin_amdgcn_readfirstlane(tid >> 6) == 0) ok = gmw_wait_head(gmw_head_crit(sy), (unsigned)ha.ncrit, &sy->abort) ? 1 : 0;
+            if (__builtin_amdgcn_readfirstlane(tid >> 6) == 0) ok = (ha.start ? gmw_wait_head(gmw_head_crit0(sy), (unsigned)ha.ncrit0, &sy->abort) : gmw_wait_head(gmw_head_crit(sy), (unsigned)ha.ncrit, &sy->abort)) ? 1 : 0;
             __syncthreads();
             head_ok = ok != 0;
             __syncthreads();
         }
         GMW_TS(sy, 128, 1);
-        if (head_ok) gmw_pivot_persist(n, ld, T, Tp, eps, G, pans, Dall, Sout, sy, ebase, Lr, Wc, facreg, xreg, keepreg, &ok, &halfcnt, stageok, tid, krows);
+        const bool hstart = ha.ntiles > 0 && ha.start != 0;
+        if (head_ok) gmw_pivot_persist(n, ld, T, Tp, eps, G, pans, Dall, Sout, sy, ebase, Lr, Wc, facreg, xreg, keepreg, &ok, &halfcnt, stageok, tid, krows,
+                                       hstart ? gmw_head_crit(sy) : nullptr, (unsigned)(ha.ncrit - ha.ncrit0), hstart);
         else if (__builtin_amdgcn_readfirstlane(tid >> 6) == 0) gmw_abandon(sy, 2);
         GMW_TS(sy, 128, 2);
     } else {
@@ -594,7 +622,11 @@
         if (role == 1) GMW_TS(sy, 129, 1);
         if (role == nmain - 1) GMW_TS(sy, 130, 1);
         if (ha.ntiles > 0) {
-            if (wv0) ok = (gmw_wait_head(gmw_head_crit(sy), (unsigned)ha.ncrit, &sy->abort) && gmw_wait_head(gmw_head_done(sy), (unsigned)(ha.ntiles - ha.ncrit), &sy->abort)) ? 1 : 0;
+            if (wv0) {
+                const unsigned int c0 = ha.start ? (unsigned)ha.ncrit0 : 0u;
+                ok = ((c0 == 0 || gmw_wait_head(gmw_head_crit0(sy), c0, &sy->abort)) && gmw_wait_head(gmw_head_crit(sy), (unsigned)ha.ncrit - c0, &sy->abort) &&
+                      gmw_wait_head(gmw_head_done(sy), (unsigned)(ha.ntiles - ha.ncrit), &sy->abort)) ? 1 : 0;
+            }
             __syncthreads();
             good = ok != 0;
             if (!good && wv0) gmw_abandon(sy, 3);
@@ -627,6 +659,7 @@
             __hip_atomic_store(&sy->exited, 0u, __ATOMIC_RELAXED, __HIP_MEMORY_SCOPE_AGENT);
             __hip_atomic_store(gmw_head_done(sy), 0u, __ATOMIC_RELAXED, __HIP_MEMORY_SCOPE_AGENT);
             __hip_atomic_store(gmw_head_crit(sy), 0u, __ATOMIC_RELAXED, __HIP_MEMORY_SCOPE_AGENT);
+            __hip_atomic_store(gmw_head_crit0(sy), 0u, __ATOMIC_RELAXED, __HIP_MEMORY_SCOPE_AGENT);
             __hip_atomic_store(&sy->resident, 0u, __ATOMIC_RELAXED, __HIP_MEMORY_SCOPE_AGENT);
             __hip_atomic_store(&sy->epoch, (ebase >> GMW_EPOCH_SHIFT) + 1, __ATOMIC_RELAXED, __HIP_MEMORY_SCOPE_AGENT);
             if (gated) atomicSub(&g_gmw_admitted, 1);
diff --git a/cv-monoslam_amd/csrc/srukf_rank.h b/cv-monoslam_amd/csrc/srukf_rank.h
--- a/cv-monoslam_amd/csrc/srukf_rank.h
+++ b/cv-monoslam_amd/csrc/srukf_rank.h
@@ -28,7 +28,8 @@
 
 struct HeadArgs {
     const int2* tiles; int ntiles;
-    int ncrit;
+    int ncrit, ncrit0;
+    int start;
     const double* dxp; double* X; const double* xr1; int ndx;
     int ngd;
     int nhelp;
diff --git a/cv-monoslam_amd/csrc/srukf_replay.hip b/cv-monoslam_amd/csrc/srukf_replay.hip
--- a/cv-monoslam_amd/csrc/srukf_replay.hip
+++ b/cv-monoslam_amd/csrc/srukf_replay.hip
@@ -324,6 +324,7 @@
             HeadArgs ha = {};
             if (head_fold) {
                 ha.tiles = (const int2*)c->syrk_head_tiles; ha.ntiles = c->n_syrk_head_tiles; ha.ncrit = c->n_syrk_head_crit;
+                ha.ncrit0 = c->n_syrk_head_crit0; ha.start = c->dbg.head_start;
                 ha.dxp = dx_src(c); ha.X = c->X; ha.xr1 = take_xr1(c); ha.ndx = c->dx_pending ? (n + 255) / 256 : 0;
                 ha.ra = rank_args(c, table, false, fuse && storage_f32_like(c)); ha.ngd = (n - c->red_r + SRUKF_RANK_COLS - 1) / SRUKF_RANK_COLS;
                 ha.nhelp = ha.ntiles + ha.ndx + ha.ngd;
```

Result: no change. 5560 frames/s, median of 6 (+0.2%).
